# razorx89/nmfgpu

Measured on AMD Instinct MI355X. Metric: NMF MU iterations/sec, dense 10kx5k r=64, higher is better.
Workload: dtype f32; 1 GPU; configs[1]: dense random V 10000x5000, r=64, MU Frobenius, fp32; rows=10000, columns=5000, features=64, error_every=10, parallelism=single GPU

## Files before the change

nmfgpu_amd/csrc/amd_api.cpp:

```cpp
#include <hip/hip_runtime.h>

#include <algorithm>
#include <cmath>
#include <cstring>
#include <string>
#include <memory>
#include <new>
#include <vector>

#include "../../include/nmfgpu_amd.h"
#include "comm.h"
#include "engine.h"
#include "tuning.h"
#include "host_init.h"
#include "sharded.h"

using namespace nmfamd;

struct nmfamd_engine {
	int elem_bytes;
	std::unique_ptr<Engine<float>> f;
	std::unique_ptr<Engine<double>> d;
};

// ... 515 lines not shown
	const int RP = padded_rank(r);
	const long Xp = pad128(X), Yp = pad128(Y);
	const int KS = (Y + 15) / 16;
	FactorProductPlan plan; plan.th = 128; plan.xtiles = (int)(Xp / 128); plan.steps_total = KS; plan.nb = 2; plan.chunks = 1;
	plan.splits = plan_splits_x3(plan.xtiles, KS, prop.multiProcessorCount);
	DevBuf dA, dT, dF, dFb, dS, dO;
	const long slab_stride = (long)RP * Xp;
	if (dA.alloc(sizeof(float) * Xp * Yp) != hipSuccess || dT.alloc(sizeof(float) * Xp * Yp) != hipSuccess || dF.alloc(sizeof(float) * RP * Yp) != hipSuccess ||
	    dFb.alloc(3 * 16 * (size_t)(KS + 1) * (RP / 32) * 64) != hipSuccess ||
	    dS.alloc(sizeof(float) * slab_stride * plan.splits) != hipSuccess || dO.alloc(sizeof(float) * slab_stride) != hipSuccess) return NMFAMD_NO_DEVICE_MEMORY;
	if (hipMemset(dA.p, 0, sizeof(float) * Xp * Yp) != hipSuccess || hipMemset(dT.p, 0, sizeof(float) * Xp * Yp) != hipSuccess ||
	    hipMemset(dF.p, 0, sizeof(float) * RP * Yp) != hipSuccess) return NMFAMD_HIP_ERROR;
	if (hipMemcpy2D(dA.p, Xp * sizeof(float), A, lda * sizeof(float), X * sizeof(float), Y, hipMemcpyHostToDevice) != hipSuccess) return NMFAMD_HIP_ERROR;
	if (hipMemcpy2D(dF.p, RP * sizeof(float), F, ldf * sizeof(float), r * sizeof(float), Y, hipMemcpyHostToDevice) != hipSuccess) return NMFAMD_HIP_ERROR;
	const int ith = (y_tiled || x16) ? 16 : 128;
	const long tstride = y_tiled ? 16 * Xp : (x16 ? 16 * Yp : 128 * Yp);
	if (y_tiled) { if (launch_tile_transposed<float>((const float*)dA.p, Xp, X, Y, (float*)dT.p, tstride, 16, nullptr) != hipSuccess) return NMFAMD_HIP_ERROR; }
	else if (launch_tile<float>((const float*)dA.p, Xp, X, Y, (float*)dT.p, tstride, ith, false, nullptr) != hipSuccess) return NMFAMD_HIP_ERROR;
	if (launch_pack_panel_x3((const float*)dF.p, RP, Y, dFb.p, KS, nullptr) != hipSuccess) return NMFAMD_HIP_ERROR;
	if (launch_factor_product_x3(plan, (const float*)dT.p, tstride, dFb.p, RP, (float*)dS.p, slab_stride, nullptr, nullptr, nullptr, y_tiled, ith) != hipSuccess) return NMFAMD_HIP_ERROR;
	if (launch_reduce_slabs<float>((const float*)dS.p, plan.splits, slab_stride, (float*)dO.p, slab_stride, nullptr) != hipSuccess) return NMFAMD_HIP_ERROR;
	if (hipMemcpy2D(OUT, ldo * sizeof(float), dO.p, RP * sizeof(float), r * sizeof(float), X, hipMemcpyDeviceToHost) != hipSuccess) return NMFAMD_HIP_ERROR;
	if (reps > 0 && avg_us) {
		DevBuf dT2;
		if (dT2.alloc(sizeof(float) * Xp * Yp) != hipSuccess) return NMFAMD_NO_DEVICE_MEMORY;
		if (hipMemcpy(dT2.p, dT.p, sizeof(float) * Xp * Yp, hipMemcpyDeviceToDevice) != hipSuccess) return NMFAMD_HIP_ERROR;
		hipEvent_t e0, e1;
		if (hipEventCreate(&e0) != hipSuccess || hipEventCreate(&e1) != hipSuccess) return NMFAMD_HIP_ERROR;
		for (int i = 0; i < 4; ++i) (void)launch_factor_product_x3(plan, (const float*)((i & 1) ? dT2.p : dT.p), tstride, dFb.p, RP, (float*)dS.p, slab_stride, nullptr, nullptr, nullptr, y_tiled, ith);
		(void)hipEventRecord(e0, nullptr);
		for (int i = 0; i < reps; ++i) (void)launch_factor_product_x3(plan, (const float*)((i & 1) ? dT2.p : dT.p), tstride, dFb.p, RP, (float*)dS.p, slab_stride, nullptr, nullptr, nullptr, y_tiled, ith);
		(void)hipEventRecord(e1, nullptr);
		if (hipEventSynchronize(e1) != hipSuccess) return NMFAMD_HIP_ERROR;
		float ms = 0; (void)hipEventElapsedTime(&ms, e0, e1);
		*avg_us = ms * 1e3 / reps;
		(void)hipEventDestroy(e0); (void)hipEventDestroy(e1);
	}
	return hipDeviceSynchronize() == hipSuccess ? NMFAMD_OK : NMFAMD_HIP_ERROR;
}

int nmfamd_op_factor_product_x3(const float* A, long lda, int X, int Y, const float* F, long ldf, int r, float* OUT, long ldo, int reps, double* avg_us) {
	return op_factor_product_x3(A, lda, X, Y, F, ldf, r, OUT, ldo, reps, avg_us, false);
}

int nmfamd_op_factor_product_x3_ytiled(const float* A, long lda, int X, int Y, const float* F, long ldf, int r, float* OUT, long ldo, int reps, double* avg_us) {
	return op_factor_product_x3(A, lda, X, Y, F, ldf, r, OUT, ldo, reps, avg_us, true);
}


int nmfamd_tune_factor_product_x3(int X, int Y, unsigned long long* stamps_out, long stamps_capacity, long* waves) {
	if (X <= 0 || Y <= 0 || !stamps_out || !waves) return NMFAMD_INVALID_ARGUMENT;
	if (nmfamd_device_count() <= 0) return NMFAMD_NO_DEVICE;
	int dev = 0; hipDeviceProp_t prop;
	if (hipGetDevice(&dev) != hipSuccess || hipGetDeviceProperties(&prop, dev) != hipSuccess) return NMFAMD_HIP_ERROR;
	const int RP = 64;
	const long Mp = pad128(X), Np = pad128(Y);
	const int ksW = (Y + 15) / 16, ksH = (X + 15) / 16;
	FactorProductPlan planW, planH;
	planW.th = planH.th = 128; planW.nb = planH.nb = 2; planW.chunks = planH.chunks = 1;
	planW.xtiles = (int)(Mp / 128); planW.steps_total = ksW; planW.splits = plan_splits_x3(planW.xtiles, ksW, prop.multiProcessorCount);
	planH.xtiles = (int)(Np / 128); planH.steps_total = ksH; planH.splits = plan_splits_x3(planH.xtiles, ksH, prop.multiProcessorCount);
	const char* ve = tuning_env("NMFAMD_X3_VARIANT");
	const bool ytiled = ve != nullptr && std::atoi(ve) >= 30;
	const FactorProductPlan& sp = ytiled ? planH : planW;
	const long nwaves = (long)sp.xtiles * sp.splits * 4;
	if (stamps_capacity < 8 * nwaves) return NMFAMD_INVALID_ARGUMENT;
	DevBuf dA, dW, dH, dWx, dHx, dS, dT;
	const long slab_stride = (long)RP * std::max(Mp, Np);
	if (dA.alloc(sizeof(float) * Mp * Np) != hipSuccess || dW.alloc(sizeof(float) * RP * Mp) != hipSuccess || dH.alloc(sizeof(float) * RP * Np) != hipSuccess ||
	    dWx.alloc(3 * 16 * (size_t)(ksH + 1) * (RP / 32) * 64) != hipSuccess || dHx.alloc(3 * 16 * (size_t)(ksW + 1) * (RP / 32) * 64) != hipSuccess ||
	    dS.alloc(sizeof(float) * slab_stride * std::max(planW.splits, planH.splits)) != hipSuccess ||
	    dT.alloc(sizeof(unsigned long long) * 8 * nwaves) != hipSuccess) return NMFAMD_NO_DEVICE_MEMORY;
	if (launch_fill_uniform<float>((float*)dA.p, (int)Mp, (int)Mp, Np, Np, 1, nullptr) != hipSuccess) return NMFAMD_HIP_ERROR;
	if (launch_fill_uniform<float>((float*)dW.p, RP, RP, Mp, Mp, 2, nullptr) != hipSuccess) return NMFAMD_HIP_ERROR;
	if (launch_fill_uniform<float>((float*)dH.p, RP, RP, Np, Np, 3, nullptr) != hipSuccess) return NMFAMD_HIP_ERROR;
	if (launch_pack_panel_x3((const float*)dW.p, RP, X, dWx.p, ksH, nullptr) != hipSuccess) return NMFAMD_HIP_ERROR;
	if (launch_pack_panel_x3((const float*)dH.p, RP, Y, dHx.p, ksW, nullptr) != hipSuccess) return NMFAMD_HIP_ERROR;
	if (hipMemset(dT.p, 0, sizeof(unsigned long long) * 8 * nwaves) != hipSuccess) return NMFAMD_HIP_ERROR;
	const long stride = 16 * Np;
	for (int i = 0; i < 40; ++i) {
		const bool last = i == 39;
		unsigned long long* sy = last && ytiled ? (unsigned long long*)dT.p : nullptr;
		unsigned long long* sx = last && !ytiled ? (unsigned long long*)dT.p : nullptr;
		if (launch_factor_product_x3(planH, (const float*)dA.p, stride, dWx.p, RP, (float*)dS.p, slab_stride, nullptr, nullptr, sy, true, 16) != hipSuccess) return NMFAMD_HIP_ERROR;
		if (launch_factor_product_x3(planW, (const float*)dA.p, stride, dHx.p, RP, (float*)dS.p, slab_stride, nullptr, nullptr, sx, false, 16) != hipSuccess) return NMFAMD_HIP_ERROR;
	}
	if (hipMemcpy(stamps_out, dT.p, sizeof(unsigned long long) * 8 * nwaves, hipMemcpyDeviceToHost) != hipSuccess) return NMFAMD_HIP_ERROR;
	*waves = nwaves;
	return NMFAMD_OK;
}

int nmfamd_op_factor_product_f64(const double* A, long lda, int X, int Y, const double* F, long ldf, int r, double* OUT, long ldo, int use_valu, int* out_slabs) {
	return op_factor_product<double>(A, lda, X, Y, F, ldf, r, OUT, ldo, use_valu != 0, out_slabs);
}

int nmfamd_op_gram_f32(const float* P, long ldp, int r, int len, float* G, long ldg) {
	if (!P || !G || r <= 0 || len <= 0 || ldp < r || ldg < r) return NMFAMD_INVALID_ARGUMENT;
	if (nmfamd_device_count() <= 0) return NMFAMD_NO_DEVICE;
	const int RP = padded_rank(r), parts = 128;
	const long lp = pad128(len);
	DevBuf dP, dPart, dG;
	if (dP.alloc(sizeof(float) * RP * lp) != hipSuccess || dPart.alloc(sizeof(float) * (size_t)RP * RP * parts) != hipSuccess || dG.alloc(sizeof(float) * RP * RP) != hipSuccess) return NMFAMD_NO_DEVICE_MEMORY;
	if (hipMemset(dP.p, 0, sizeof(float) * RP * lp) != hipSuccess) return NMFAMD_HIP_ERROR;
	if (hipMemcpy2D(dP.p, RP * sizeof(float), P, ldp * sizeof(float), r * sizeof(float), len, hipMemcpyHostToDevice) != hipSuccess) return NMFAMD_HIP_ERROR;
	if (launch_gram<float>((const float*)dP.p, RP, len, parts, (float*)dPart.p, (float*)dG.p, nullptr) != hipSuccess) return NMFAMD_HIP_ERROR;
	if (hipMemcpy2D(G, ldg * sizeof(float), dG.p, RP * sizeof(float), r * sizeof(float), r, hipMemcpyDeviceToHost) != hipSuccess) return NMFAMD_HIP_ERROR;
	return hipDeviceSynchronize() == hipSuccess ? NMFAMD_OK : NMFAMD_HIP_ERROR;
}

int nmfamd_op_gram_f64(const double* P, long ldp, int r, int len, double* G, long ldg) {
	if (!P || !G || r <= 0 || len <= 0 || ldp < r || ldg < r) return NMFAMD_INVALID_ARGUMENT;
	if (nmfamd_device_count() <= 0) return NMFAMD_NO_DEVICE;
	const int RP = padded_rank(r, sizeof(double)), parts = 128;
	const long lp = pad128(len);
	DevBuf dP, dPart, dG;
	if (dP.alloc(sizeof(double) * RP * lp) != hipSuccess || dPart.alloc(sizeof(double) * (size_t)RP * RP * parts) != hipSuccess || dG.alloc(sizeof(double) * RP * RP) != hipSuccess) return NMFAMD_NO_DEVICE_MEMORY;
	if (hipMemcpy2D(dP.p, RP * sizeof(double), P, ldp * sizeof(double), r * sizeof(double), len, hipMemcpyHostToDevice) != hipSuccess) return NMFAMD_HIP_ERROR;
	if (launch_gram<double>((const double*)dP.p, RP, len, parts, (double*)dPart.p, (double*)dG.p, nullptr) != hipSuccess) return NMFAMD_HIP_ERROR;
	if (hipMemcpy2D(G, ldg * sizeof(double), dG.p, RP * sizeof(double), r * sizeof(double), r, hipMemcpyDeviceToHost) != hipSuccess) return NMFAMD_HIP_ERROR;
	return hipDeviceSynchronize() == hipSuccess ? NMFAMD_OK : NMFAMD_HIP_ERROR;
}

int nmfamd_op_inverse_f32(const float* A, long lda, int r, float offdiag, float diag, float* Ainv, long ldi) {
	if (!A || !Ainv || r <= 0 || lda < r || ldi < r) return NMFAMD_INVALID_ARGUMENT;
	if (nmfamd_device_count() <= 0) return NMFAMD_NO_DEVICE;
	const int RP = padded_rank(r);
	DevBuf dA, dI, dW;
	if (dA.alloc(sizeof(float) * RP * RP) != hipSuccess || dI.alloc(sizeof(float) * RP * RP) != hipSuccess || dW.alloc(sizeof(double) * 2 * (size_t)r * r) != hipSuccess) return NMFAMD_NO_DEVICE_MEMORY;
	if (hipMemcpy2D(dA.p, RP * sizeof(float), A, lda * sizeof(float), r * sizeof(float), r, hipMemcpyHostToDevice) != hipSuccess) return NMFAMD_HIP_ERROR;
	if (launch_inverse_small<float>((float*)dA.p, RP, r, (float*)dI.p, (double*)dW.p, offdiag, diag, nullptr) != hipSuccess) return NMFAMD_HIP_ERROR;
	if (hipMemcpy2D(Ainv, ldi * sizeof(float), dI.p, RP * sizeof(float), r * sizeof(float), r, hipMemcpyDeviceToHost) != hipSuccess) return NMFAMD_HIP_ERROR;
	return hipDeviceSynchronize() == hipSuccess ? NMFAMD_OK : NMFAMD_HIP_ERROR;
}

int nmfamd_op_tri_update_f32(const float* P, const float* num, const float* Q, int r, int len, const float* old_colsq, int transform_num, const float* num_colsq,
                             float theta, float frag_theta, int transform_den, float* P_out, float* pack_out, float* scale_out, float* gram_out,
                             float* gram_raw_out, float* gram_image_out, float* diag_out) {
	if (!P || !num || !Q || r <= 0 || len <= 0) return NMFAMD_INVALID_ARGUMENT;
	if (nmfamd_device_count() <= 0) return NMFAMD_NO_DEVICE;
	const int RP = padded_rank(r);
	if (!tri_kernels_available(RP)) return NMFAMD_INVALID_ARGUMENT;
	const long lp = pad128(len), KS = (len + 15) / 16;
	const size_t pack_bytes = 16 * (size_t)KS * (RP / 32) * 64;
	int dev = 0, cus = 256;
	hipDeviceProp_t prop;
	if (hipGetDevice(&dev) == hipSuccess && hipGetDeviceProperties(&prop, dev) == hipSuccess && prop.multiProcessorCount > 0) cus = prop.multiProcessorCount;
	const int parts = panel_update_parts(RP, sizeof(float), (int)lp);
	DevBuf dP, dN, dQ, dOs, dNs, dPack, dPart, dG, dSq, dStage, dScale, dQx, dDummy, dG2, dImg, dDiag;
	const size_t img_bytes = (size_t)3 * 16 * (RP / 16 + 1) * (RP / 32) * 64;
	if (dG2.alloc(sizeof(float) * RP * RP) != hipSuccess || dImg.alloc(img_bytes) != hipSuccess || dDiag.alloc(sizeof(float) * RP) != hipSuccess) return NMFAMD_NO_DEVICE_MEMORY;
	if (dP.alloc(sizeof(float) * RP * lp) != hipSuccess || dN.alloc(sizeof(float) * RP * lp) != hipSuccess || dQ.alloc(sizeof(float) * RP * RP) != hipSuccess ||
	    dOs.alloc(sizeof(float) * RP) != hipSuccess || dNs.alloc(sizeof(float) * RP) != hipSuccess || dPack.alloc(pack_bytes) != hipSuccess ||
	    dPart.alloc(sizeof(float) * (size_t)gram_tri_partial_elems(cus)) != hipSuccess || dG.alloc(sizeof(float) * RP * RP) != hipSuccess ||
	    dSq.alloc(sizeof(float) * ((size_t)parts + 16) * RP) != hipSuccess || dStage.alloc(sizeof(float) * RP * colsq_stage_parts()) != hipSuccess ||
	    dScale.alloc(sizeof(float) * RP) != hipSuccess || dDummy.alloc(sizeof(float) * RP * 4) != hipSuccess || dQx.alloc((size_t)3 * 16 * (RP / 16 + 1) * (RP / 32) * 64) != hipSuccess) return NMFAMD_NO_DEVICE_MEMORY;
	if (hipMemcpy2D(dP.p, RP * sizeof(float), P, r * sizeof(float), r * sizeof(float), len, hipMemcpyHostToDevice) != hipSuccess) return NMFAMD_HIP_ERROR;
	if (hipMemcpy2D(dN.p, RP * sizeof(float), num, r * sizeof(float), r * sizeof(float), len, hipMemcpyHostToDevice) != hipSuccess) return NMFAMD_HIP_ERROR;
	if (hipMemcpy2D(dQ.p, RP * sizeof(float), Q, r * sizeof(float), r * sizeof(float), r, hipMemcpyHostToDevice) != hipSuccess) return NMFAMD_HIP_ERROR;
	if (old_colsq && hipMemcpy(dOs.p, old_colsq, sizeof(float) * r, hipMemcpyHostToDevice) != hipSuccess) return NMFAMD_HIP_ERROR;
	if (num_colsq && hipMemcpy(dNs.p, num_colsq, sizeof(float) * r, hipMemcpyHostToDevice) != hipSuccess) return NMFAMD_HIP_ERROR;
	PanelTriExtras ex;
	ex.num_transform = transform_num != 0;
	ex.num_colsq = num_colsq ? (const float*)dNs.p : nullptr; ex.num_colsq_parts = 1;
	const float off = theta / (float)(unsigned)r, diag = (float)((1.0 - theta) + off);
	ex.num_a = diag - off; ex.num_b = off; ex.r = r;
	ex.old_colsq = old_colsq ? (const float*)dOs.p : nullptr; ex.old_colsq_parts = 1;
	ex.frag_out = dPack.p; ex.frag_KS = KS;
// ... 254 lines not shown
```

nmfgpu_amd/csrc/engine.cpp:

```cpp
#include "engine.h"
#include "tuning.h"

#include <algorithm>
#include <cmath>
#include <cstdint>
#include <cstdio>
#include <cstdlib>
#include <cstring>
#include <limits>
#include <type_traits>

namespace nmfamd {

#define HIPX(call)                                        \
	do {                                                  \
		hipError_t e__ = (call);                          \
		if (e__ != hipSuccess) return hip_fail(e__, #call); \
	} while (0)

template <typename T>
double resolve_frobenius(const std::vector<T>& vtv_sorted, std::vector<T>& htwtv, std::vector<T>& hhtwtw) {
	return std::sqrt(resolve_frobenius_squared<T>(vtv_sorted, htwtv, hhtwtw));
}
template double resolve_frobenius<float>(const std::vector<float>&, std::vector<float>&, std::vector<float>&);
// ... 161 lines not shown
		if (why != nullptr) { last_error_ = why; return ST_INVALID; }
		tiled_ = false;
		planH_.splits = planW_.splits = 1; planH_.th = planW_.th = 128;
		planH_.xtiles = (int)(pad128(n_) / 128); planW_.xtiles = (int)(pad128(m_) / 128);
	}
	if (beta_dense_) {
		tiled_ = false;
		planH_.th = planW_.th = 128;
		planH_.xtiles = (int)(pad128(n_) / 128); planW_.xtiles = (int)(pad128(m_) / 128);
		betaH_ = plan_beta_half_step(pad128(n_), pad128(m_), RP_, sizeof(T), num_cus_);
		betaW_ = plan_beta_half_step(pad128(m_), pad128(n_), RP_, sizeof(T), num_cus_);
		planH_.splits = betaH_.slabs; planW_.splits = betaW_.slabs;
	}
	if (prm_.precision > 0) {
		if (!std::is_same<T, float>::value || sparse_ || !mfma) return ST_INVALID;
		bf16_ = true;
		tiled_ = false;
		planH_.th = planW_.th = 128;
		planH_.xtiles = (int)(pad128(n_) / 128); planW_.xtiles = (int)(pad128(m_) / 128);
		ksW_ = (n_ + 15) / 16; ksH_ = (m_ + 15) / 16;
		planH_.splits = plan_splits_bf16(planH_.xtiles, ksH_, RP_, num_cus_);
		planW_.splits = plan_splits_bf16(planW_.xtiles, ksW_, RP_, num_cus_);
		if (RP_ == 256 && (alg_ == ALG_MU || alg_ == ALG_NSNMF) && tri_kernels_available(RP_)) {
			const char* e = tuning_env("NMFAMD_TRI_RIDE");
			const bool want_w = e == nullptr || (e[0] != '0' && e[0] != 'h'), want_h = e == nullptr || (e[0] != '0' && e[0] != 'w');
			if (want_w && num_cus_ > 2 * TRI_PASSENGERS) {
				FactorProductPlan t = planH_;
				t.splits = plan_splits_bf16(planH_.xtiles, ksH_, RP_, num_cus_ - TRI_PASSENGERS);
				if (bf16_product_workgroups(t) + TRI_PASSENGERS <= num_cus_) { planH_.splits = t.splits; tri_ride_w_ = true; }
			}
			tri_ride_h_ = want_h && bf16_product_workgroups(planW_) + TRI_PASSENGERS <= num_cus_;
		}
		planHb_ = planH_; planWb_ = planW_;
	}
	const size_t image_bytes = sizeof(T) * (size_t)pad128(m_) * (size_t)pad128(n_);
	const size_t mall = memory_side_cache_bytes(prop);
	const bool cache_window = mall > 0 && (double)image_bytes > 0.6 * (double)mall && (double)image_bytes < 1.12 * (double)mall && std::getenv("NMFAMD_ONE_IMAGE") == nullptr;
#ifdef NMFAMD_DIAG_BUILD
	const char* op_env = tuning_env("NMFAMD_ONE_PASS");
	const bool op_req = op_env != nullptr && std::atoi(op_env) != 0 && one_pass_allowed_ && row_blocks_ == 1 && fused_capable() && RP_ == 64 &&
	                    std::getenv("NMFAMD_GRAM_PARTIALS") == nullptr && tuning_env("NMFAMD_IMAGE_TILE128") == nullptr && onepass_available(pad128(m_), num_cus_);
#else
	const bool op_req = false;
#endif
	if (std::is_same<T, float>::value && tiled_ && !bf16_ && !sparse_ && RP_ % 64 == 0 && prm_.precision == 0 && (planH_.nb == 2 || cache_window || op_req) &&
	    tuning_env("NMFAMD_FP32_NATIVE") == nullptr) {
		planH_.nb = planW_.nb = 2;
		x3_ = true;
		planH_.th = planW_.th = 128;
		planH_.xtiles = (int)(pad128(n_) / 128); planW_.xtiles = (int)(pad128(m_) / 128);
		ksW_ = (n_ + 15) / 16; ksH_ = (m_ + 15) / 16;
		gram_ksplit_ = 1;
		if (fused_capable() && RP_ == 64 && std::getenv("NMFAMD_GRAM_PARTIALS") == nullptr) {
			const double product_us = 6.0 + (double)sizeof(T) * (double)pad128(m_) * (double)pad128(n_) / 5.0e6;
			const double pairs = (ksH_ + 2) / 2;
			while (gram_ksplit_ < GRAM_KSPLIT_MAX && 24.0 * (pairs / 317.0) / gram_ksplit_ > 0.55 * product_us) gram_ksplit_ *= 2;
			if (const char* e = tuning_env("NMFAMD_GRAM_KSPLIT")) { const int k = std::atoi(e); if (k == 1 || k == 2 || k == 4 || k == 8) gram_ksplit_ = k; }
		}
		planH_.splits = plan_splits_x3(planH_.xtiles, ksH_, num_cus_, gram_ksplit_ > 1 ? GRAM_IMAGE_TILES * gram_ksplit_ : 0);
		planW_.splits = plan_splits_x3(planW_.xtiles, ksW_, num_cus_);
		planHx_ = planH_; planWx_ = planW_;
		planHx_.steps_total = ksH_; planWx_.steps_total = ksW_;
		planHx_.nb = planWx_.nb = 2;
		size_t free_b = 0, total_b = 0;
		const size_t image_b = sizeof(T) * (size_t)pad128(m_) * (size_t)pad128(n_);
		const char* force = std::getenv("NMFAMD_ONE_IMAGE");
		one_pass_ = op_req && (force == nullptr || std::atoi(force) != 0);
		if (one_pass_) one_image_ = true;
		else if (force != nullptr) one_image_ = std::atoi(force) != 0;
		else if (cache_window) one_image_ = true;
		else if (hipMemGetInfo(&free_b, &total_b) == hipSuccess && 3 * image_b + (image_b >> 3) > free_b) one_image_ = true;
		w_col_split_ = false;
		if (RP_ == 64 && fused_capable() && !one_image_ && 2 * planW_.xtiles + GRAM_REDUCE_BLOCKS <= 2 * num_cus_) {
			w_col_split_ = ksW_ <= 80 && 4 * planW_.xtiles >= num_cus_;
			if (const char* e = tuning_env("NMFAMD_X3_COLSPLIT")) { const int v = std::atoi(e); if (v == 0) w_col_split_ = false; else if (v == 1) w_col_split_ = true; }
			if (w_col_split_) { planW_.splits = planWx_.splits = 1; planWx_.col_split = 2; }
		}
		if (const char* e = tuning_env("NMFAMD_X3_COLSPLIT")) { if (std::atoi(e) == 2 && RP_ == 64 && fused_capable()) { planHx_.col_split = planWx_.col_split = 2; w_col_split_ = true; } }
	}
	mpad_ = pad128(std::max<long>(m_, (long)planW_.xtiles * planW_.th));
	if (row_blocks_ > 1) { const long g = 128l * row_blocks_; mpad_ = ((mpad_ + g - 1) / g) * g; }
	npad_ = pad128(std::max<long>(n_, (long)planH_.xtiles * planH_.th));
	img_th_ = (one_image_ && tuning_env("NMFAMD_IMAGE_TILE128") == nullptr) ? 16 : planW_.th;
	strideV_ = (long)img_th_ * npad_;
	strideVt_ = (long)planH_.th * mpad_;
	elemsV_ = mpad_ * npad_;
	elemsVt_ = tiled_ ? (long)planH_.xtiles * strideVt_ : mpad_ * npad_;
	slab_stride_ = (long)RP_ * std::max(mpad_, npad_);
	const long slab_elems = slab_stride_ * std::max(planH_.splits, planW_.splits);
	const long panelW = (long)RP_ * mpad_, panelH = (long)RP_ * npad_, rr = (long)RP_ * RP_;

	auto dalloc = [&](T** p, long elems) -> hipError_t {
		hipError_t e = hipMalloc((void**)p, (size_t)elems * sizeof(T));
		if (e != hipSuccess) return e;
		return hipMemsetAsync(*p, 0, (size_t)elems * sizeof(T), stream_);
	};
	if (bf16_) {
		HIPX(hipMalloc(&Vb_, 16 * (size_t)planW_.xtiles * ksW_ * 256));
		HIPX(hipMalloc(&Vtb_, 16 * (size_t)planH_.xtiles * ksH_ * 256));
		{
			const size_t ks_alloc = (size_t)std::max<long>(ksH_, mpad_ / 16);
			HIPX(hipMalloc(&Wtb_, 16 * ks_alloc * (RP_ / 32) * 64));
			if (ks_alloc > (size_t)ksH_) HIPX(hipMemsetAsync((char*)Wtb_ + 16 * (size_t)ksH_ * (RP_ / 32) * 64, 0, 16 * (ks_alloc - (size_t)ksH_) * (RP_ / 32) * 64, stream_));
		}
		HIPX(hipMalloc(&Hb_, 16 * (size_t)ksW_ * (RP_ / 32) * 64));
	} else if (!sparse_) {
		if (x3_) {
			const size_t bw = 3 * 16 * (size_t)(ksH_ + 1) * (RP_ / 32) * 64, bh = 3 * 16 * (size_t)(ksW_ + 1) * (RP_ / 32) * 64;
			HIPX(hipMalloc(&Wx3_, bw));
			HIPX(hipMalloc(&Hx3_, bh));
			HIPX(hipMemsetAsync(Wx3_, 0, bw, stream_));
			HIPX(hipMemsetAsync(Hx3_, 0, bh, stream_));
		}
		HIPX(dalloc(&V_, elemsV_));
		if (!one_image_) HIPX(dalloc(&Vt_, elemsVt_));
	} else {
		HIPX(dalloc(&t_vwh_, mpad_));
		HIPX(dalloc(&t_kl_, mpad_));
		HIPX(dalloc(&rowsum_part_, (std::max(mpad_, npad_) / 128) * RP_));
		HIPX(dalloc(&sW_, RP_));
		HIPX(dalloc(&sH_, RP_));
		HIPX(dalloc(&kl_scale_, RP_));
		HIPX(hipHostMalloc((void**)&pin_kl_, sizeof(T) * (2 * (size_t)m_ + 3 * (size_t)RP_)));
		if (prm_.is_masked()) HIPX(dalloc(&msq_part_, (long)(MASKED_NORM_PARTS + 16) * RP_));
	}
	if (beta_dense_) {
		HIPX(dalloc(&t_vwh_, mpad_));
		HIPX(dalloc(&t_kl_, mpad_));
		HIPX(dalloc(&rowsum_part_, (std::max(mpad_, npad_) / 128) * RP_));
		HIPX(dalloc(&sW_, RP_));
		HIPX(dalloc(&sH_, RP_));
		HIPX(dalloc(&beta_tpart_, 2l * BETA_MAX_SLABS * mpad_));
		if (beta_ != 1) HIPX(dalloc(&beta_den_, slab_elems));
		HIPX(hipHostMalloc((void**)&pin_kl_, sizeof(T) * (2 * (size_t)m_ + 3 * (size_t)RP_)));
	}
	HIPX(dalloc(&Wt_, panelW));
	HIPX(dalloc(&H_, panelH));
	if (std::is_same<T, float>::value && panel_update_wide_available(RP_) && std::getenv("NMFAMD_FORCE_VALU") == nullptr &&
	    tuning_env("NMFAMD_WIDE_FP32_MFMA") == nullptr)
	{
		const size_t qb = 3 * 16 * (size_t)(RP_ / 16 + 1) * (RP_ / 32) * 64;
		HIPX(hipMalloc(&qx3_, qb));
		HIPX(hipMemsetAsync(qx3_, 0, qb, stream_));
	}
	HIPX(dalloc(&slabs_, slab_elems));
	HIPX(dalloc(&numW_, panelW));
	HIPX(dalloc(&G_, rr));
	HIPX(dalloc(&G2_, rr));
	HIPX(dalloc(&HHt_, rr));
	HIPX(dalloc(&Qinv_, rr));
	HIPX(dalloc(&gram_part_, rr * gram_parts_));
	HIPX(dalloc(&sumsq_part_, ((long)std::max({panel_update_parts(RP_, sizeof(T), (int)mpad_), (int)(mpad_ / panel_update_rows(RP_, sizeof(T))),
	                                           alg_ == ALG_HALS ? panel_sweep_hals_parts(RP_, sizeof(T), (int)mpad_) : 0}) + 16) * RP_));
	ps_stride_ = std::max<long>(npad_, RP_);
	HIPX(dalloc(&psN_, ps_stride_ + RP_));
	psR_ = psN_ + ps_stride_;
	HIPX(dalloc(&stage_, std::max(mpad_, npad_) * RP_));
	HIPX(hipMalloc((void**)&range_flag_, sizeof(int)));
	if constexpr (std::is_same<T, float>::value) {
		tri_ = bf16_ && tri_kernels_available(RP_) && (alg_ == ALG_MU || alg_ == ALG_NSNMF);
		if (tri_) {
			HIPX(hipMalloc((void**)&gram_tri_part_, sizeof(float) * (size_t)std::max<long>(gram_tri_partial_elems(num_cus_), (long)(TRI_PASSENGERS / 2) * 36 * 1024)));
			HIPX(hipMalloc((void**)&tri_ride_counters_, 64));
			HIPX(hipMemsetAsync(tri_ride_counters_, 0, 64, stream_));
			HIPX(dalloc(&Gw_raw_, rr));
			HIPX(dalloc(&Gh_raw_, rr));
// ... 406 lines not shown
void Engine<T>::record_begin(int kind) {
	if (!timing_ || !timing_now_) return;
	if (ev_used_ + 2 > ev_.size()) {
		for (int i = 0; i < 64; ++i) { hipEvent_t e; if (hipEventCreate(&e) != hipSuccess) return; ev_.push_back(e); }
	}
	if (ev_kind_.size() < ev_.size() / 2) ev_kind_.resize(ev_.size() / 2, 0);
	ev_kind_[ev_used_ / 2] = (char)kind;
	(void)hipEventRecord(ev_[ev_used_], stream_);
}

template <typename T>
bool Engine<T>::timed_launch_events(int kind, hipEvent_t* start, hipEvent_t* stop) {
	*start = *stop = nullptr;
	if (!timing_ || !timing_now_) return false;
	if (ev_used_ + 2 > ev_.size()) {
		for (int i = 0; i < 64; ++i) { hipEvent_t e; if (hipEventCreate(&e) != hipSuccess) return false; ev_.push_back(e); }
	}
	if (ev_kind_.size() < ev_.size() / 2) ev_kind_.resize(ev_.size() / 2, 0);
	ev_kind_[ev_used_ / 2] = (char)kind;
	*start = ev_[ev_used_]; *stop = ev_[ev_used_ + 1];
	return true;
}

template <typename T>
void Engine<T>::record_end() {
	if (!timing_ || !timing_now_ || ev_used_ + 2 > ev_.size()) return;
	(void)hipEventRecord(ev_[ev_used_ + 1], stream_);
	ev_used_ += 2;
}

template <typename T>
void Engine<T>::dominant_stats(double* total_ms, long* launches, double* pair_overhead_ms, double* kind_ms, long* kind_launches) {
	double tot = 0; long cnt = 0;
	double km[2] = {0, 0}; long kc[2] = {0, 0};
	(void)hipStreamSynchronize(stream_);
	for (size_t i = 0; i + 1 < ev_used_; i += 2) {
		float ms = 0;
		if (hipEventElapsedTime(&ms, ev_[i], ev_[i + 1]) == hipSuccess) {
			tot += ms; ++cnt;
			const int k = (i / 2 < ev_kind_.size() && ev_kind_[i / 2] != 0) ? 1 : 0;
			km[k] += ms; ++kc[k];
		}
	}
	ev_used_ = 0;
	if (total_ms) *total_ms = tot;
	if (launches) *launches = cnt;
	if (kind_ms) { kind_ms[0] = km[0]; kind_ms[1] = km[1]; }
	if (kind_launches) { kind_launches[0] = kc[0]; kind_launches[1] = kc[1]; }
	if (pair_overhead_ms) {
		double best = -1;
		if (ev_.size() >= 2) {
			for (int i = 0; i < 8; ++i) {
				(void)hipEventRecord(ev_[0], stream_);
				(void)hipEventRecord(ev_[1], stream_);
				(void)hipEventSynchronize(ev_[1]);
				float ms = 0;
				if (hipEventElapsedTime(&ms, ev_[0], ev_[1]) == hipSuccess && (best < 0 || ms < best)) best = ms;
			}
		}
		*pair_overhead_ms = best < 0 ? 0.0 : best;
	}
}

template <typename T>
GramReduceArgs Engine<T>::gram_args(bool of_w, float* G, float* scale, int normalize) const {
	GramReduceArgs rg = {of_w ? gramW_part_ : gramH_part_, (int)((of_w ? mpad_ : npad_) / 64), G, scale, normalize};
	if (gram_image_) {
		rg.partials = nullptr; rg.parts = 0; rg.image = of_w ? Wx3_ : Hx3_; rg.image_ks = of_w ? ksH_ : ksW_;
		if (of_w && normalize != 0 && wsq_part_ != nullptr) { rg.colsq_part = wsq_part_; rg.colsq_parts = (int)(mpad_ / 32); }
		if (of_w && (const void*)G == (const void*)G_ && gram_ksplit_ > 1 && Gpart_ != nullptr && (normalize == 0 || rg.colsq_part != nullptr)) { rg.ksplit = gram_ksplit_; rg.G = Gpart_; }
		else if (of_w && (const void*)G == (const void*)G_ && gram_spread_ && Gpart_ != nullptr && (normalize == 0 || rg.colsq_part != nullptr)) { rg.spread = 1; rg.G = Gpart_; rg.spread_out = G; rg.spread_counter = gram_spread_counter_; }
	}
	return rg;
}

template <typename T>
Status Engine<T>::standalone_gram(const GramReduceArgs& rg) {
	if (rg.image != nullptr) HIPX(launch_gram_image_args(rg, stream_));
	else HIPX(launch_mu64_gram_reduce(rg, stream_));
	return ST_OK;
}

template <typename T>
Status Engine<T>::mu64_update(bool is_w, const T* slabs, int S, long slab_stride, const T* Q, bool compute_error, const PeerSlabs* peers) {
	if constexpr (std::is_same<T, float>::value) {
		const float eps = std::numeric_limits<float>::epsilon();
		float* P = is_w ? Wt_ : H_;
		float* ps = ps_direct_ ? (is_w ? pin_psN_dev_ + ps_stride_ : pin_psN_dev_) : (is_w ? psR_ : psN_);
		const int len = is_w ? m_ : n_, len_pad = (int)(is_w ? mpad_ : npad_);
		void* xo = x3_ ? (is_w ? Wx3_ : Hx3_) : nullptr;
		const int xks = is_w ? ksH_ : ksW_;
		if (peers != nullptr && !gram_image_) return ST_INVALID;
		SmoothAround ns;
		ns.off = (float)prm_.theta / (float)(unsigned)r_; ns.diag = (float)((1.0 - (float)prm_.theta) + ns.off); ns.r = r_;
		const bool smooth = alg_ == ALG_NSNMF && !is_w;
		if (alg_ == ALG_NSNMF && !gram_image_) return ST_INVALID;
		if (gram_image_) HIPX(launch_mu64_update32(is_w ? 1 : 0, P, slabs, S, slab_stride, Q, scale_, eps, ps, len, len_pad, is_w ? G_ : nullptr, compute_error ? 1 : 0, stream_, xo, xks, peers,
		                                           is_w ? wsq_part_ : nullptr, (!is_w && (const void*)Q == (const void*)Gpart_) ? gram_ksplit_ : 0, (!is_w && (const void*)Q == (const void*)Gpart_) ? G_ : nullptr,
		                                           smooth ? &ns : nullptr));
		else HIPX(launch_mu64_update(is_w ? 1 : 0, P, slabs, S, slab_stride, Q, scale_, eps, ps, len, len_pad, is_w ? gramW_part_ : gramH_part_, is_w ? G_ : nullptr,
		                             compute_error ? 1 : 0, stream_, xo, xks));
	}
	return ST_OK;
}

template <typename T>
Status Engine<T>::product_h(const T* F, const GramReduceArgs* rg, bool prepacked) {
	if (sparse_) {
		if (rg) { if (Status st = standalone_gram(*rg)) return st; }
		record_begin();
		HIPX(launch_spmm_rows<T>(csc_ptr_, csc_idx_, csc_val_, F, RP_, slabs_, n_, (int)npad_, stream_));
		record_end();
		return ST_OK;
	}
	if constexpr (std::is_same<T, float>::value) {
		if (bf16_) {
			if (!prepacked) HIPX(launch_pack_panel_bf16(F, RP_, m_, Wtb_, ksH_, stream_));
			if (rg && rg->tri_frags == nullptr && planHb_.xtiles < GRAM_REDUCE_BLOCKS) { if (Status st = standalone_gram(*rg)) return st; rg = nullptr; }
			record_begin();
#ifdef NMFAMD_DIAG_BUILD
			if (unsigned long long* st = bf_stamps(0)) set_factor_product_bf16_stamps(st);
#endif
			HIPX(launch_factor_product_bf16(planHb_, Vtb_, ksH_, Wtb_, RP_, slabs_, slab_stride_, stream_, rg));
			record_end();
			return ST_OK;
		}
		if (x3_) {
			if (!prepacked) HIPX(launch_pack_panel_x3(F, RP_, m_, Wx3_, ksH_, stream_));
			if (rg && rg->wide_P == nullptr && !passengers_ride(planHx_)) { if (Status st = standalone_gram(*rg)) return st; rg = nullptr; }
			hipEvent_t e0, e1;
			const bool timed = timed_launch_events(0, &e0, &e1);
			if (one_image_) HIPX(launch_factor_product_x3(planHx_, V_, strideV_, Wx3_, RP_, slabs_, slab_stride_, stream_, rg, nullptr, true, img_th_, e0, e1));
			else HIPX(launch_factor_product_x3(planHx_, Vt_, strideVt_, Wx3_, RP_, slabs_, slab_stride_, stream_, rg, nullptr, false, 128, e0, e1));
			if (timed) timed_launch_done();
			return ST_OK;
		}
		if (tiled_) {
			if (rg && planH_.xtiles < GRAM_REDUCE_BLOCKS) { if (Status st = standalone_gram(*rg)) return st; rg = nullptr; }
			record_begin();
			HIPX(launch_factor_product_f32(planH_, Vt_, strideVt_, F, RP_, slabs_, slab_stride_, stream_, rg));
			record_end();
			return ST_OK;
		}
	}
	if constexpr (std::is_same<T, double>::value) {
		if (tiled_) {
			record_begin();
			HIPX(launch_factor_product_f64(planH_, Vt_, strideVt_, F, RP_, slabs_, slab_stride_, stream_, ride64_));
			record_end();
			return ST_OK;
		}
	}
	record_begin();
	HIPX(launch_factor_product_valu<T>(Vt_, npad_, (int)npad_, m_, F, RP_, slabs_, stream_));
	record_end();
	return ST_OK;
}

template <typename T>
Status Engine<T>::product_w(const T* F, const GramReduceArgs* rg, T* single_slab_out, bool prepacked) {
	T* dest = (single_slab_out != nullptr && planW_.splits == 1) ? single_slab_out : slabs_;
	if (sparse_) {
		if (rg) { if (Status st = standalone_gram(*rg)) return st; }
		record_begin(1);
		HIPX(launch_spmm_rows<T>(csr_ptr_, csr_idx_, csr_val_, F, RP_, dest, m_, (int)mpad_, stream_));
		record_end();
		return ST_OK;
	}
	if constexpr (std::is_same<T, float>::value) {
		if (bf16_) {
			if (!prepacked) HIPX(launch_pack_panel_bf16(F, RP_, n_, Hb_, ksW_, stream_));
			if (rg && rg->tri_frags == nullptr && planWb_.xtiles < GRAM_REDUCE_BLOCKS) { if (Status st = standalone_gram(*rg)) return st; rg = nullptr; }
			record_begin(1);
#ifdef NMFAMD_DIAG_BUILD
			if (unsigned long long* st = bf_stamps(1)) set_factor_product_bf16_stamps(st);
#endif
			HIPX(launch_factor_product_bf16(planWb_, Vb_, ksW_, Hb_, RP_, dest, slab_stride_, stream_, rg));
			record_end();
			return ST_OK;
		}
		if (x3_) {
			if (!prepacked) HIPX(launch_pack_panel_x3(F, RP_, n_, Hx3_, ksW_, stream_));
// ... 735 lines not shown
#ifdef NMFAMD_DIAG_BUILD
	if constexpr (std::is_same<T, float>::value) {
		if (!fused_ready_) { normalize_next_ = 0; fused_ready_ = true; }
		if (!wx3_valid_) { HIPX(launch_pack_panel_x3(Wt_, RP_, m_, Wx3_, ksH_, stream_)); wx3_valid_ = true; }
		GramReduceArgs rgW = gram_args(true, G_, scale_, normalize_next_);
		rgW.ksplit = 0; rgW.spread = 0; rgW.G = G_;
		if (Status s = standalone_gram(rgW)) return s;
		OnePassArgs a;
		a.V = V_; a.tile_stride = strideV_;
		a.Wx3 = Wx3_; a.G = G_; a.scale = scale_; a.ps = op_ps4_; a.ps_stride = npad_;
		if constexpr (std::is_same<T, float>::value) { a.H = H_; a.H_out = op_H2_; }
		a.slabs = op_slabs_; a.slab_stride = (long)RP_ * mpad_;
		a.hh_part = op_hh_part_; a.part_scratch = op_part_; a.hfrag_scratch = op_hfrag_;
		a.ticket = op_ctl_; a.abort_flag = op_ctl_ + 8;
		a.tile_rows = (int)(mpad_ / 16); a.w_ks = ksH_; a.n = n_; a.panels = (n_ + 31) / 32;
		a.seq = op_seq_++;
		a.compute_error = compute_error ? 1 : 0;
		a.eps = std::numeric_limits<float>::epsilon();
		a.stamps = op_stamps_;
		record_begin();
#ifdef NMFAMD_DIAG_BUILD
		HIPX(launch_mu64_onepass(a, stream_));
#else
		return ST_INVALID;
#endif
		record_end();
		std::swap(H_, op_H2_);
		HIPX(launch_reduce_partials<float>(op_hh_part_, ONEPASS_XCDS * ONEPASS_GROUP, 4096, HHt_, 4096, stream_));
		if (compute_error) HIPX(launch_reduce_partials<float>(op_ps4_, 4, npad_, psN_, n_, stream_));
		if (Status s = mu64_update(true, op_slabs_, ONEPASS_XCDS, (long)RP_ * mpad_, HHt_, compute_error)) return s;
		wx3_valid_ = x3_;
		hx3_valid_ = false;
		normalize_next_ = 1;
		w_pending_ = true;
		if (compute_error) {
			if (Status s = fetch_error_terms(n_)) return s;
			if (Status s = onepass_check()) return s;
		}
	}
#else
	(void)compute_error;
#endif
	return ST_OK;
}

template <typename T>
Status Engine<T>::onepass_check() {
#ifdef NMFAMD_DIAG_BUILD

	HIPX(hipMemcpyAsync(pin_abort_, op_ctl_ + 8, sizeof(unsigned), hipMemcpyDeviceToHost, stream_));
	HIPX(hipStreamSynchronize(stream_));
	if (op_stamps_ != nullptr) {
		std::vector<unsigned long long> h(16 * 8 * ONEPASS_XCDS * ONEPASS_GROUP);
		if (hipMemcpy(h.data(), op_stamps_, sizeof(unsigned long long) * h.size(), hipMemcpyDeviceToHost) == hipSuccess) {
			if (FILE* f = std::fopen(tuning_env("NMFAMD_ONEPASS_STAMPS"), "wb")) { std::fwrite(h.data(), sizeof(unsigned long long), h.size(), f); std::fclose(f); }
		}
	}
	if (*pin_abort_ != 0) {
		one_pass_ = false; one_pass_gave_up_ = true;
		last_error_ = "the one-pass iteration could not keep its workgroups resident (another kernel on the device?): factors are void; unset NMFAMD_ONE_PASS";
		return ST_HIP_ERROR;
	}
#endif
	return ST_OK;
}

template <typename T>
Status Engine<T>::iterate_mu64(bool compute_error) {
	if constexpr (std::is_same<T, float>::value) {
		if (one_pass_) return iterate_onepass(compute_error);
		const float eps = std::numeric_limits<float>::epsilon();
		static const bool no_direct = tuning_env("NMFAMD_ERROR_MEMCPY") != nullptr || tuning_env("NMFAMD_ERROR_COPY_KERNEL") != nullptr;
		ps_direct_ = compute_error && gram_image_ && !error_terms_stay_ && pin_psN_dev_ != nullptr && !no_direct;
		if (ps_direct_) finalize_error(false);
		struct DirectGuard { bool& f; ~DirectGuard() { f = false; } } direct_guard{ps_direct_};
		if (!fused_ready_) {
			if (!gram_image_) HIPX(launch_mu64_gram_partials(Wt_, (int)mpad_, gramW_part_, stream_));
			normalize_next_ = 0;
			fused_ready_ = true;
		}
		GramReduceArgs rgW = gram_args(true, G_, scale_, normalize_next_);
		if (h_product_ahead_) h_product_ahead_ = false;
		else if (Status s = product_h(Wt_, &rgW, x3_ && wx3_valid_)) return s;
		if (Status s = mu64_update(false, slabs_, planH_.splits, slab_stride_, rgW.ksplit > 1 ? reinterpret_cast<const T*>(Gpart_) : G_, compute_error)) return s;
		GramReduceArgs rgH = gram_args(false, HHt_, nullptr, 0);
		if (Status s = product_w(H_, &rgH, nullptr, x3_)) return s;
		if (Status s = mu64_update(true, slabs_, planW_.splits, slab_stride_, HHt_, compute_error)) return s;
		wx3_valid_ = x3_;
		hx3_valid_ = false;
		normalize_next_ = 1;
		w_pending_ = true;
		if (compute_error) {
			if (Status s = fetch_error_terms(n_)) return s;
		}
	}
	return ST_OK;
}

template <typename T>
Status Engine<T>::begin_next_iteration() {
	if constexpr (std::is_same<T, double>::value) {
		if (!fused64_capable() || f64_partial_ == nullptr || !f64_pending_ || f64_product_ahead_ || prm_.divergence != 0) return ST_OK;
		const bool sampled = timing_now_;
		timing_now_ = false;
		const Status s = fused64_product_h();
		timing_now_ = sampled;
		if (s != ST_OK) return s;
		f64_product_ahead_ = true;
		return ST_OK;
	}
	if constexpr (std::is_same<T, float>::value) {
		if (!fused_capable() || one_pass_ || !fused_ready_ || h_product_ahead_ || prm_.divergence != 0 || !x3_ || !wx3_valid_) return ST_OK;
		GramReduceArgs rgW = gram_args(true, G_, scale_, normalize_next_);
		const bool sampled = timing_now_;
		timing_now_ = false;
		const Status s = product_h(Wt_, &rgW, true);
		timing_now_ = sampled;
		if (s != ST_OK) return s;
		h_product_ahead_ = true;
	}
	return ST_OK;
}

template <typename T>
Status Engine<T>::set_hals_penalties(double l1W, double l1H, double l2W, double l2H) {
	if (const char* why = hals_penalties_fault(l1W, l1H, l2W, l2H, sizeof(T) == 4, prm_.takes_penalties(alg_ == ALG_HALS))) { last_error_ = why; return ST_INVALID; }
	prm_.l1W = (double)(T)l1W; prm_.l1H = (double)(T)l1H; prm_.l2W = (double)(T)l2W; prm_.l2H = (double)(T)l2H;
	return ST_OK;
}

template <typename T>
Status Engine<T>::iterate(bool compute_error, bool constant_w) {
	const T eps = std::numeric_limits<T>::epsilon();
	timing_now_ = timing_ && (timing_iter_++ % timing_stride_ == 0);
	if (prm_.is_masked()) return iterate_masked(compute_error, constant_w);
	if (beta_dense_) return iterate_beta(compute_error, constant_w);
	if (prm_.divergence != 0) return constant_w ? ST_INVALID : iterate_kl(compute_error);
	if (fused_capable() && !constant_w) return iterate_mu64(compute_error);
	if (fused64_capable() && !constant_w) return iterate_fused64(compute_error);
	if (f32w_scale_ != nullptr && fused32w_capable() && !constant_w) return iterate_fused32w(compute_error);
	const int norm_parts = panel_update_parts(RP_, sizeof(T), (int)mpad_);
	h_partials_unneeded_ = !constant_w;
	const Status hs = h_step_impl(compute_error);
	h_partials_unneeded_ = false;
	if (hs != ST_OK) return hs;

	const bool ls_family = alg_ == ALG_ALS || alg_ == ALG_ACLS || alg_ == ALG_AHCLS;
	int error_terms_n = n_;

	if (!(constant_w && !compute_error)) {
		const T* Fh = H_;
		bool hht_done = false;
		GramReduceArgs tri_ride = {nullptr, 0, nullptr, nullptr, 0};
		if (tri_) {
			if (Status s = tri_prepare_h(HHt_, true, !constant_w ? &tri_ride : nullptr)) return s;
			hht_done = true;
		} else if (alg_ == ALG_NSNMF) {
			const T off = (T)prm_.theta / (T)(unsigned)r_;
			const T diag = (T)((1.0 - (T)prm_.theta) + off);
			HIPX(launch_smooth_panel<T>(H_, Hs_, RP_, r_, npad_, off, diag, stream_));
			Fh = Hs_;
		}
		bool hht_rides = false;
		if constexpr (std::is_same<T, float>::value) {
			hht_rides = !constant_w && alg_ == ALG_GDCLS && x3_ && hx3_valid_ && Fh == H_ && RP_ == 64 && !gram_h_partials_ && passengers_ride(planWx_);
			if (!hht_rides && gram_h_partials_ && Fh == H_) {
				HIPX(launch_gram64_from_partials(gramH_part_, (int)(npad_ / 64), HHt_, nullptr, stream_));
				hht_done = true;
			}
		}
// ... 481 lines not shown
```

nmfgpu_amd/csrc/engine.h:

```cpp
#pragma once

#include <hip/hip_runtime.h>
#include <stdint.h>

#include <functional>
#include <vector>

#include "kernels.h"

namespace nmfamd {

enum Algorithm { ALG_MU = 0, ALG_GDCLS = 1, ALG_ALS = 2, ALG_ACLS = 3, ALG_AHCLS = 4, ALG_NSNMF = 5, ALG_HALS = 6 };

struct AlgorithmParams {
	double lambda = 0, lambdaW = 0, lambdaH = 0, alphaW = 0, alphaH = 0, theta = 0;
	double divergence = 0;
	double sparse_compute = 0;
	double precision = 0;
	double missing_values = 0;
	double l1W = 0, l1H = 0, l2W = 0, l2H = 0;
	double dense_compute = 0;
	double beta_value = 0;
	bool is_masked() const { return missing_values != 0; }
	bool is_beta_dense() const { return divergence == 2 || divergence == 3 || (divergence == 1 && dense_compute != 0); }
// ... 116 lines not shown
	int n() const { return n_; }
	int r() const { return r_; }
	int rp() const { return RP_; }
	bool error_terms_per_factor_row() const { return alg_ != ALG_MU && alg_ != ALG_NSNMF && alg_ != ALG_HALS; }
	int algorithm() const { return alg_; }
	long mpad() const { return mpad_; }
	long npad() const { return npad_; }
	int slabs_h() const { return planH_.splits; }
	int slabs_w() const { return planW_.splits; }
	int resident_images() const { return sparse_ ? 0 : (one_image_ ? 1 : 2); }
	int product_kernel() const { return beta_dense_ ? 6 : sparse_ ? 5 : bf16_ ? 1 : x3_ ? 2 : !tiled_ ? 4 : (sizeof(T) == 8 ? 3 : 0); }
	const char* last_error() const { return last_error_; }

	Status debug_read(int which, T* out, long count);

private:
	Status hip_fail(hipError_t e, const char* what);
	Status h_step_impl(bool compute_error);
	Status product_h(const T* F, const GramReduceArgs* rg = nullptr, bool prepacked = false);
	Status product_w(const T* F, const GramReduceArgs* rg = nullptr, T* single_slab_out = nullptr, bool prepacked = false);
	bool fused_capable() const;
	bool fused32w_capable() const;
	Status iterate_fused32w(bool compute_error);
	bool fused64_capable() const;
	Status iterate_fused64(bool compute_error);
	bool gram_from_update() const;
	Status iterate_mu64(bool compute_error);
	Status iterate_onepass(bool compute_error);
	Status onepass_check();
	Status materialize_w(bool whole_panel = true);
	Status ensure_w_rows();
	Status normalize_w(bool from_gram_partials, int norm_parts);
	Status normal_inverse(T* A, T offdiag, T diag);
	Status normal_inverse_fork(T* A, T offdiag, T diag);
	Status normal_inverse_join();
	bool passengers_ride(const FactorProductPlan& plan) const;
	bool inverse_rides(const FactorProductPlan& plan) const;
	Status finish_upload(T* Vcol);
	Status upload_triplets(std::vector<int>& rows, std::vector<int>& cols, std::vector<T>& vals);
	Status upload_sparse_device(int format, const T* values, const int* a, const int* b, long nnz, int base, bool* fallback);
	Status setup_kl_blocks();
	bool sparse_setup_on_device_ = false;
	Status iterate_kl(bool compute_error);
	Status iterate_masked(bool compute_error, bool constant_w);
	Status masked_refuses(const char* what);
	Status iterate_beta(bool compute_error, bool constant_w);
	Status beta_refuses(const char* what);
	Status beta_check_values(const T* values, long count, long ld, long rows);
	Status fetch_error_terms(int count_n);
	void finalize_error(bool resolve);
	void record_begin(int kind = 0);
	void record_end();
	bool timed_launch_events(int kind, hipEvent_t* start, hipEvent_t* stop);
	void timed_launch_done() { ev_used_ += 2; }

	int m_, n_, r_, RP_, alg_;
	int row_blocks_ = 1;
	AlgorithmParams prm_;
	long mpad_, npad_;
	long strideV_ = 0, strideVt_ = 0, elemsV_ = 0, elemsVt_ = 0;
	int num_cus_ = 256;
	hipStream_t stream_ = nullptr;
	hipStream_t aux_ = nullptr;
	hipEvent_t ev_fork_ = nullptr, ev_join_ = nullptr;
	bool overlap_inverse_ = false;
	bool tiled_ = false;
	const char* last_error_ = "";

	T *V_ = nullptr, *Vt_ = nullptr;
	T *Wt_ = nullptr, *H_ = nullptr;
	T *Ws_ = nullptr, *Hs_ = nullptr;
	T *slabs_ = nullptr;
	T *numW_ = nullptr;
	T *Wold_ = nullptr;
	T *rowdot_part_ = nullptr;
	T *G_ = nullptr, *G2_ = nullptr, *HHt_ = nullptr, *Qinv_ = nullptr, *gram_part_ = nullptr;
	T *sumsq_part_ = nullptr;
	bool bf16_ = false;
	void *Vb_ = nullptr, *Vtb_ = nullptr, *Wtb_ = nullptr, *Hb_ = nullptr;
	int ksW_ = 0, ksH_ = 0;
	FactorProductPlan planHb_, planWb_;
	bool x3_ = false;
	bool one_image_ = false;
	int img_th_ = 128;
	bool wx3_valid_ = false, hx3_valid_ = false;
	void *Wx3_ = nullptr, *Hx3_ = nullptr;
	void* qx3_ = nullptr;
	FactorProductPlan planHx_, planWx_;
	bool sparse_ = false;
	long nnz_ = 0;
	int *csr_ptr_ = nullptr, *csr_idx_ = nullptr, *csc_ptr_ = nullptr, *csc_idx_ = nullptr, *csc_from_csr_ = nullptr;
	T *csr_val_ = nullptr, *csc_val_ = nullptr, *q_ = nullptr, *q2_ = nullptr;
	T *t_vwh_ = nullptr, *t_kl_ = nullptr, *rowsum_part_ = nullptr, *sW_ = nullptr, *sH_ = nullptr;
	int kl_blocks_w_ = 1, kl_blocks_h_ = 1;
	int *csr_bptr_ = nullptr, *csc_bptr_ = nullptr;
	T *kl_part_ = nullptr, *kl_tpart_ = nullptr;
	double sum_v_ = 0, kl_ = 0;
	T* pin_kl_ = nullptr;
	bool kl_pending_ = false, kl_unresolved_ = false;
	std::vector<T> h_klrow_, h_sW_, h_sH_;
	T* msq_part_ = nullptr;
	bool masked_pending_ = false, masked_unresolved_ = false;
	bool beta_dense_ = false, beta_uploaded_ = false;
	double beta_ = 1;
	BetaPlan betaH_, betaW_;
	T *beta_den_ = nullptr, *beta_tpart_ = nullptr;
	bool beta_pending_ = false, beta_unresolved_ = false;
	float *gramW_part_ = nullptr, *gramH_part_ = nullptr, *scale_ = nullptr, *Graw64_ = nullptr;
	bool w_col_split_ = false;
	bool gram_spread_ = false;
	unsigned* gram_spread_counter_ = nullptr;
	int gram_ksplit_ = 1;
	float* Gpart_ = nullptr;
	float* wsq_part_ = nullptr;
	bool fused_ready_ = false, w_pending_ = false;
	bool h_product_ahead_ = false;
	bool gram_image_ = false;
	GramReduceArgs gram_args(bool of_w, float* G, float* scale, int normalize) const;
	Status standalone_gram(const GramReduceArgs& rg);
	Status mu64_update(bool is_w, const T* slabs, int S, long slab_stride, const T* Q, bool compute_error, const PeerSlabs* peers = nullptr);
	bool gram_w_ready_ = false;
	bool tri_ = false;
	unsigned* tri_ride_counters_ = nullptr;
	bool tri_ride_w_ = false, tri_ride_h_ = false;
	bool wtb_valid_ = false;
	bool tri_scale_pending_ = false;
	bool tri_scale_from_gram_ = false;
	bool sole_rank_ = false;
	T* kl_scale_ = nullptr;
	bool kl_scale_pending_ = false;
	bool kl_sw_ready_ = false;
	bool kl_err_iter_ = false;
	long err_total_columns_ = 0;
	Status kl_h_step();
	Status kl_w_products(T* exchange, bool compute_error);
	Status kl_w_finish(const T* exchange, bool compute_error);
	bool tri_w_den_bf16_ = true;
	bool hb_valid_ = false;
	const T* tri_trace_scale() const { return (tri_ && tri_scale_pending_) ? reinterpret_cast<const T*>(colsq_) : nullptr; }
	bool tri_gw_ready_ = false;
	bool tri_rows_cover_ = false;
	bool w_rows_stale_ = false;
	std::function<Status()> w_gather_hook_;
	int colsq_parts_ = 1;
	float *gram_tri_part_ = nullptr, *Gw_raw_ = nullptr, *Gh_raw_ = nullptr, *colsq_ = nullptr;
	bool qx3_holds_g_ = false, qx3_holds_hht_ = false;
	void tri_smoothing(T* offdiag, T* diag) const;
	Status tri_prepare_w(GramReduceArgs* ride = nullptr);
	Status tri_prepare_h(T* hht, bool local_q, GramReduceArgs* ride = nullptr);
	Status tri_update_w(const T* num, int S, long stride, const T* hht);
	bool f32w_pending_ = false;
	float* f32w_scale_ = nullptr;
	int f32w_ride_h_ = 0, f32w_ride_w_ = 0;
	bool f64_pending_ = false;
	bool f64_product_ahead_ = false;
	Status fused64_product_h();
	double *f64_scale_ = nullptr, *f64_partial_ = nullptr;
	unsigned* f64_counters_ = nullptr;
	int *f64_items_h_ = nullptr, *f64_items_w_ = nullptr;
	int f64_slices_h_ = 0, f64_slices_w_ = 0;
	const GramRideF64* ride64_ = nullptr;
	unsigned long long* f64_stamps_ = nullptr;
	bool gram_h_partials_ = false;
	bool h_partials_unneeded_ = false;
	int normalize_next_ = 0;
	T *psN_ = nullptr, *psR_ = nullptr;
	long ps_stride_ = 0;
	double* inv_work_ = nullptr;
	T* stage_ = nullptr;
	int* range_flag_ = nullptr;
	long slab_stride_ = 0;
	int gram_parts_ = 128;
	FactorProductPlan planH_, planW_;
	bool one_pass_allowed_ = true, one_pass_ = false, one_pass_gave_up_ = false;
	void *op_part_ = nullptr, *op_hfrag_ = nullptr;
	unsigned *op_ctl_ = nullptr;
	float *op_slabs_ = nullptr, *op_hh_part_ = nullptr, *op_ps4_ = nullptr;
	T* op_H2_ = nullptr;
	unsigned op_seq_ = 0;
	unsigned* pin_abort_ = nullptr;
	unsigned long long* op_stamps_ = nullptr;

	T *pin_psN_ = nullptr, *pin_psR_ = nullptr;
	bool error_terms_stay_ = false;
	bool ps_last_direct_ = false;
	bool ps_direct_ = false;
	T* pin_psN_dev_ = nullptr;
	hipEvent_t err_event_ = nullptr;
	bool err_pending_ = false, err_unresolved_ = false;
	int err_count_ = 0;
	std::vector<T> h_vtv_, h_psN_, h_psR_;
	double frob_ = 0, frob2_ = 0, rmsd_ = 0;

	bool timing_ = false;
	int timing_stride_ = 1;
	long timing_iter_ = 0;
	bool timing_now_ = false;
	std::vector<hipEvent_t> ev_;
	std::vector<char> ev_kind_;
	size_t ev_used_ = 0;
};

template <typename T>
// ... 6 lines not shown
```

nmfgpu_amd/csrc/kernels.h:

```cpp
#pragma once

#include <hip/hip_runtime.h>
#include <stddef.h>
#include <stdint.h>

#include <atomic>
#include <vector>

namespace nmfamd {

struct FactorProductPlan {
	int th;
	int xtiles;
	int steps_total;
	int splits;
	int nb;
	int chunks;
	int xhalves = 0;
	int half_tiles = 0;
	int col_split = 0;
};

FactorProductPlan plan_factor_product(int X, int Y, int RP, int num_cus);

inline hipError_t allow_dynamic_lds(const void* kernel, int bytes, std::atomic<unsigned long long>& done) {
	int dev = 0;
	hipError_t e = hipGetDevice(&dev);
	if (e != hipSuccess) return e;
	if (dev >= 0 && dev < 64 && ((done.load(std::memory_order_acquire) >> dev) & 1ull)) return hipSuccess;
	e = hipFuncSetAttribute(kernel, hipFuncAttributeMaxDynamicSharedMemorySize, bytes);
	if (e == hipSuccess && dev >= 0 && dev < 64) done.fetch_or(1ull << dev, std::memory_order_release);
	return e;
}

struct GramReduceArgs {
	const float* partials;
	int parts;
	float* G;
	float* scale;
	int normalize;
	const float* inv_a = nullptr;
	float* inv_out = nullptr;
	float inv_offdiag = 0.f, inv_diag = 0.f;
	int inv_r = 0;
	const void* image = nullptr;
	int image_ks = 0;
	const float* colsq_part = nullptr;
	int colsq_parts = 0;
	int ksplit = 0;
	int spread = 0;
	float* spread_out = nullptr;
	unsigned* spread_counter = nullptr;
	const void* tri_frags = nullptr;
	int tri_ks = 0;
	void* tri_x3 = nullptr;
	float* tri_diag = nullptr;
	float* tri_partial = nullptr;
	unsigned* tri_counters = nullptr;
	const float* wide_P = nullptr;
	int wide_len = 0, wide_parts = 0;
	float* wide_partial = nullptr;
};
constexpr int GRAM_REDUCE_BLOCKS = 16;
constexpr int TRI_PASSENGERS = 32;
constexpr int GRAM_IMAGE_TILES = 10;
constexpr int GRAM_SPREAD_SLICES = 3;
constexpr int GRAM_KSPLIT_MAX = 8;

hipError_t launch_factor_product_f32(const FactorProductPlan& p, const float* A, long tile_stride, const float* F, int RP,
                                     float* slabs, long slab_stride, hipStream_t stream, const GramReduceArgs* rg = nullptr);

template <typename T>
hipError_t launch_tile(const T* src, long ld, int X, int Y, T* dst, long tile_stride, int th, bool untile, hipStream_t stream);
template <typename T>
hipError_t launch_tile_transposed(const T* src, long ld, int I, int J, T* dst, long tile_stride, int th, hipStream_t stream);

hipError_t launch_factor_product_f32_stamped(const FactorProductPlan& p, const float* A, long lda, const float* F, int RP,
                                             float* slabs, long slab_stride, unsigned long long* stamps, hipStream_t stream);

hipError_t launch_mu64_gram_partials(const float* P, int len_pad, float* partial, hipStream_t stream);
hipError_t launch_mu64_gram_reduce(const GramReduceArgs& rg, hipStream_t stream);
hipError_t launch_mu64_update(int is_w, float* P, const float* slabs, int S, long slab_stride, const float* Q, const float* scale,
                              float eps, float* ps, int len_valid, int len_pad, float* gram_partial, const float* Gprev,
                              int compute_error, hipStream_t stream, void* x3_out = nullptr, int x3_ks = 0);
constexpr int PEER_SLABS_MAX = 16;
struct PeerSlabs { const float* p[PEER_SLABS_MAX]; int count; };
struct SmoothAround { float off, diag; int r; };
hipError_t launch_mu64_update32(int is_w, float* P, const float* slabs, int S, long slab_stride, const float* Q, const float* scale,
                                float eps, float* ps, int len_valid, int len_pad, const float* Gprev, int compute_error, hipStream_t stream,
                                void* x3_out, int x3_ks, const PeerSlabs* peers = nullptr, float* colsq_part = nullptr, int qsplit = 0, float* q_out = nullptr,
                                const SmoothAround* ns = nullptr);
hipError_t launch_sum_peers(const PeerSlabs& src, float* out, int count, hipStream_t stream);
hipError_t launch_gram_from_image(const void* image, int image_ks, float* G, float* scale, int normalize, hipStream_t stream, const float* colsq_part = nullptr, int colsq_parts = 0);
hipError_t launch_gram_image_args(const GramReduceArgs& rg, hipStream_t stream);
hipError_t launch_mu64_apply_scale(float* P, int len_pad, const float* scale, hipStream_t stream, void* x3_out = nullptr, int x3_ks = 0);
hipError_t launch_gram64_from_partials(const float* partials, int parts, float* G, float* scale, hipStream_t stream);
hipError_t launch_gram64_normalize_all(const float* partials, int parts, float* Graw, float* G, float* scale, float* P, int len_pad, void* x3_out, int x3_ks, hipStream_t stream);
hipError_t launch_gram64_reduce_scale_all(const float* gram_part, int parts, const float* sumsq_part, int sq_parts, float* G, float* scale, float* P, int len_pad,
                                          void* x3_out, int x3_ks, hipStream_t stream);

template <typename T>
hipError_t launch_factor_product_valu(const T* A, long lda, int Xpad, int Y, const T* F, int RP, T* out, hipStream_t stream);

template <typename T>
hipError_t launch_reduce_slabs(const T* slabs, int S, long slab_stride, T* out, long count, hipStream_t stream);

template <typename T>
hipError_t launch_gram(const T* P, int RP, int len, int parts, T* partial, T* G, hipStream_t stream);

enum PanelMode { PANEL_MU = 0, PANEL_LS = 1, PANEL_SET = 2 };
struct PanelTriExtras {
	bool num_transform = false;
	const float* num_colsq = nullptr;
	int num_colsq_parts = 0;
	float num_a = 1.0f, num_b = 0.0f;
	int r = 0;
	bool den_transform = false;
	float den_a = 1.0f, den_b = 0.0f;
	const float* den_colsq = nullptr;
	int den_colsq_parts = 0;
	const float* old_colsq = nullptr;
	int old_colsq_parts = 0;
	bool old_as_bf16 = false;
	void* frag_out = nullptr;
	long frag_KS = 0;
	float frag_a = 1.0f, frag_b = 0.0f;
};
int panel_update_rows(int RP, size_t elem);
int panel_update_parts(int RP, size_t elem, int len_pad);

hipError_t launch_gram64_f32(const float* P, int len, int parts, float* partial, float* G, hipStream_t stream);
hipError_t launch_panel_update64_f32(int mode, float* P, const float* slabs, int S, long slab_stride, const float* Q, int len_pad,
                                     float eps, float* ps, int len_valid, float* sumsq_part, float* num_out, hipStream_t stream);
hipError_t launch_panel_update64_lds_f32(int mode, float* P, const float* slabs, int S, long slab_stride, const float* Q, int len_pad,
                                         float eps, float* ps, int len_valid, float* sumsq_part, float* num_out, hipStream_t stream,
                                         float* gram_partial = nullptr, void* x3_out = nullptr, int x3_ks = 0);
bool panel_update_delivers_gram(int RP, size_t elem);
bool panel_update_wide_available(int RP);
bool panel_update_long_available(int RP, int len_pad);
hipError_t launch_panel_update_long_mu(const float* P_in, float* P_out, const float* slabs, int S, long slab_stride, const void* q_split, int RP, int len_pad,
                                       float eps, float* ps, int len_valid, float* sumsq_part, hipStream_t stream, const PanelTriExtras* tri = nullptr);
bool gram_wide_available(int RP);
hipError_t launch_gram_wide_f32(const float* P, int RP, int len, int parts, float* partial, float* G, hipStream_t stream);
struct PanelFusedF32 {
	const float* old_scale = nullptr;
	int h_side = 0;
	const float* scale = nullptr;
	int smooth = 0;
	float off = 0.f, diag = 1.f;
	int r = 0;
	float* smooth_out = nullptr;
	void* x3_out = nullptr;
	long x3_ks = 0;
};
hipError_t launch_panel_update_wide_f32(int mode, float* P, const float* slabs, int S, long slab_stride, const float* Q, int RP, int len_pad,
                                        float eps, float* ps, int len_valid, float* sumsq_part, float* num_out, hipStream_t stream,
                                        void* q_split = nullptr, const PanelTriExtras* tri = nullptr, const PanelFusedF32* fused = nullptr);
hipError_t launch_gram_reduce_x3(const float* partial, int parts, int RP, float* G, void* qx3, const float* sumsq_part, int sq_parts, float* scale_out, hipStream_t stream);
int gram_wide_fused_parts(int RP, int len, int parts);
hipError_t launch_gram_wide_fused_f32(const float* P, int RP, int len, int parts, float* partial, float* G, void* qx3, const float* sumsq_part, int sq_parts,
                                      float* scale_out, hipStream_t stream);
template <typename T>
hipError_t launch_reduce_partials(const T* partial, int parts, long stride, T* out, long count, hipStream_t stream);
template <typename T>
hipError_t launch_normalize_panel_v2(T* P, int RP, int len_pad, T* sumsq_part, int parts, hipStream_t stream);

template <typename T>
hipError_t launch_panel_update(int mode, T* P, const T* slabs, int S, long slab_stride, const T* Q, int RP, int len_pad,
                               T eps, T* ps, int len_valid, T* sumsq_part, T* num_out, hipStream_t stream, T* gram_partial = nullptr,
                               void* x3_out = nullptr, int x3_ks = 0,
                               void* q_split = nullptr,
                               const PanelTriExtras* tri = nullptr);

bool panel_sweep_hals_available(int RP, size_t elem);
// ... 33 lines not shown
template <typename T>
hipError_t launch_column_sumsq(const T* V, long ldv, int rows, int cols, T* ps, hipStream_t stream, int* range_flag = nullptr);

template <typename T>
hipError_t launch_densify(int format, const T* values, const int* ptr, const int* idx, const int* idx2, long nnz, int outer, int base,
                          T* V, long ldv, int rows, int cols, hipStream_t stream);

template <typename T>
hipError_t launch_fill_uniform(T* P, int RP, int r, long len, long len_pad, uint64_t seed, hipStream_t stream, long y_first = 0);

FactorProductPlan plan_factor_product_f64(int X, int Y, int RP, int num_cus);
struct GramRideF64 {
	const double* P;
	int len;
	int slices;
	double* partial;
	unsigned* counters;
	double* G;
	const double* sumsq_part;
	int sumsq_parts;
	double* scale_out;
	const int* items;
	int stop;
	unsigned long long* stamps;
};
int gram_ride_f64_workgroups(int RP, int slices);
hipError_t launch_factor_product_f64(const FactorProductPlan& p, const double* A, long tile_stride, const double* F, int RP,
                                     double* slabs, long slab_stride, hipStream_t stream, const GramRideF64* ride = nullptr);
void gram_ride_f64_items(const FactorProductPlan& p, int RP, int slices, std::vector<int>& items);

struct PanelFusedF64 {
	const double* old_scale;
	int h_side;
	const double* scale;
	int smooth;
	double off, diag;
	int r;
	double* smooth_out;
	const double* trace_a;
	const double* trace_b;
	const double* trace_scale;
	double* trace_out;
	int trace_r;
	unsigned long long* stamps;
};
inline int panel_fused_f64_extra_workgroups(const PanelFusedF64* fx) { return (fx != nullptr && fx->trace_out != nullptr) ? (fx->trace_r + 3) / 4 : 0; }
hipError_t launch_panel_update64_f64(int mode, double* P, const double* slabs, int S, long slab_stride, const double* Q, int len_pad,
                                     double eps, double* ps, int len_valid, double* sumsq_part, double* num_out, hipStream_t stream, const PanelFusedF64* fused = nullptr);

hipError_t launch_gram_f64(const double* P, int RP, int len, int parts, double* partial, double* G, hipStream_t stream);
bool panel_update_wide_f64_available(int RP);
hipError_t launch_panel_update_wide_f64(int mode, double* P, const double* slabs, int S, long slab_stride, const double* Q, int RP, int len_pad,
                                        double eps, double* ps, int len_valid, double* sumsq_part, double* num_out, hipStream_t stream, const PanelFusedF64* fused = nullptr);

hipError_t launch_pack_stream_bf16(const float* src, long ld, int X, int Y, bool transposed, void* dst, int xtiles, int KS, hipStream_t stream);
hipError_t launch_pack_panel_bf16(const float* P, int RP, int len, void* dst, int KS, hipStream_t stream);

bool tri_kernels_available(int RP);
hipError_t launch_finish_panel_bf16(float* P, int RP, int r, long row0, long rows, const float* colsq, int colsq_parts, float offdiag, float diag, void* dst, long KS, hipStream_t stream);
int colsq_stage_parts();
hipError_t launch_colsq_stage(const float* part, int RP, int parts, float* staged, float* final_sum, hipStream_t stream);
hipError_t launch_gram_tri(const float* P, int RP, int len, int max_parts, float* partial, float* G, int num_cus, hipStream_t stream);
long gram_tri_partial_elems(int max_parts);
hipError_t launch_gram_tri_bf16(const void* frags, int RP, long KS, int max_parts, float* partial, float* G, const float* colsq, int colsq_parts, int num_cus, hipStream_t stream);
hipError_t launch_gram_tri_bf16_image(const void* frags, int RP, long KS, int max_parts, float* partial, float* G, void* x3_out, float* diag_out, int num_cus, hipStream_t stream);
hipError_t launch_scale_panel_tri(float* P, int RP, long rows, const float* colsq, int colsq_parts, float* scale_out, hipStream_t stream);
hipError_t launch_smooth_gram(const float* G, float* Gs, int RP, int r, float offdiag, float diag, void* x3_out, hipStream_t stream);
hipError_t launch_finish_and_gram(const float* P_in, float* P_out, int RP, int r, long rows, int len, const float* colsq, int colsq_parts, float offdiag, float diag,
                                  void* dst, long KS, int max_parts, float* partial, float* G, int num_cus, hipStream_t stream);
hipError_t launch_factor_product_bf16(const FactorProductPlan& p, const void* A, int KS, const void* F, int RP,
                                      float* slabs, long slab_stride, hipStream_t stream, const GramReduceArgs* rg = nullptr);
int plan_splits_bf16(int xtiles, int KS, int RP, int num_cus);
int bf16_product_workgroups(const FactorProductPlan& p);
#ifdef NMFAMD_DIAG_BUILD
void set_factor_product_bf16_stamps(unsigned long long* stamps);
#endif

hipError_t launch_pack_panel_x3(const float* P, int RP, int len, void* dst, int KS, hipStream_t stream);
hipError_t launch_factor_product_x3(const FactorProductPlan& p, const float* A, long tile_stride, const void* F, int RP,
                                    float* slabs, long slab_stride, hipStream_t stream, const GramReduceArgs* rg = nullptr,
                                    unsigned long long* stamps = nullptr, bool y_tiled = false, int image_tile = 128,
                                    hipEvent_t ev_start = nullptr, hipEvent_t ev_stop = nullptr);
int plan_splits_x3(int xtiles, int KS, int num_cus, int reserve = 0);

struct OnePassArgs {
	const float* V; long tile_stride;
	const void* Wx3;
	const float* G;
	const float* scale;
	const float* H;
	float* H_out;
	float* ps; long ps_stride;
	float* slabs; long slab_stride;
	float* hh_part;
	void* part_scratch;
	void* hfrag_scratch;
	unsigned* ticket;
	unsigned* abort_flag;
	int tile_rows;
	int w_ks;
	int n;
	int panels;
	unsigned seq;
	int compute_error;
	float eps;
	unsigned long long* stamps = nullptr;
};
constexpr int ONEPASS_SLOTS = 4;
constexpr int ONEPASS_GROUP = 32;
constexpr int ONEPASS_XCDS = 8;
constexpr int ONEPASS_TILES_PER_WAVE = 5;
constexpr size_t onepass_part_bytes() { return (size_t)ONEPASS_XCDS * ONEPASS_SLOTS * ONEPASS_GROUP * 256 * 64; }
constexpr size_t onepass_hfrag_bytes() { return (size_t)ONEPASS_XCDS * ONEPASS_SLOTS * 64 * 32 * 8; }
bool onepass_available(long mpad, int num_cus);
hipError_t launch_mu64_onepass(const OnePassArgs& a, hipStream_t stream);

template <typename T>
hipError_t launch_spmm_rows(const int* ptr, const int* idx, const T* val, const T* P, int RP, T* out, int rows, int rows_pad, hipStream_t stream);
template <typename T>
hipError_t launch_sddmm_quotient(const int* ptr, const int* idx, const T* val, const T* A, const T* B, int RP, T eps,
                                 T* q, T* t_vwh, T* t_kl, int rows, hipStream_t stream);
template <typename T>
hipError_t launch_kl_fused(const int* ptr, const int* idx, const T* val, const T* A, const T* B, int RP, T eps,
                           T* out, T* t_vwh, T* t_kl, int rows, int rows_pad, hipStream_t stream, int blocks = 1, long out_stride = 0,
                           const T* a_scale = nullptr);
template <typename T>
hipError_t launch_permute(const T* src, const int* perm, T* dst, long count, hipStream_t stream);
template <typename T>
hipError_t launch_panel_rowsum(const T* P, int RP, int len_pad, T* partial, T* sums, hipStream_t stream);
template <typename T>
hipError_t launch_kl_update(T* P, const T* num, const T* den, int RP, int len_pad, T eps, T* sumsq_part, hipStream_t stream, int parts = 1, long part_stride = 0,
                            T* sum_part = nullptr,
                            const T* scale = nullptr);
template <typename T>
hipError_t launch_kl_sums(const T* sum_part, const T* sumsq_part, int parts, int RP, T* sums, hipStream_t stream, T* scale_out = nullptr);

constexpr int MASKED_NORM_PARTS = 2048;
int masked_norm_parts(int rows);
template <typename T>
hipError_t launch_masked_half_step(const int* ptr, const int* idx, const T* val, T* A, const T* B, int RP, T eps, bool update,
                                   T* t_res, T* sumsq_part, int rows, hipStream_t stream);

constexpr int BETA_MAX_SLABS = 16;
struct BetaPlan { int bo = 0, kt = 0, slabs = 0, tiles = 0, tiles_per_slab = 0; };
bool beta_half_step_available(int RP);
BetaPlan plan_beta_half_step(long out_pad, long red_pad, int RP, size_t elem_bytes, int num_cus, int force_slabs = 0);
template <typename T>
hipError_t launch_beta_fused(const T* X, long ldx, const T* A, const T* B, int RP, double beta, bool update, bool terms, T eps, const BetaPlan& plan,
                             T* num_part, T* den_part, long part_stride, T* tf_part, T* td_part, long t_stride,
                             int out_pad, int out_valid, int red_valid, hipStream_t stream);
template <typename T>
hipError_t launch_beta_update(T* A, const T* num_part, const T* den_part, long part_stride, int slabs, const T* dsum, int RP, int r, int out_pad, int out_valid, T eps,
                              double beta, T l1, T l2, bool update, T* sumsq_part, T* sum_part, const T* tf_part, const T* td_part, long t_stride, T* t_frob,
                              T* t_div, hipStream_t stream);

hipError_t launch_sp_expand(int format, const int* a, const int* b, long nnz, int outer, int base, int m, int n, int* row, int* col, int* flags, hipStream_t stream);
hipError_t launch_sp_histogram_scan(const int* key, long count, int segments, int* counts, int* ptr, int* maxlen, hipStream_t stream);
long sp_segment_sort_capacity();
hipError_t launch_sp_scatter_sort(const int* key, long count, int segments, const int* ptr, int* fill, int* items, const int* minor, int maxlen, hipStream_t stream);
template <typename T>
hipError_t launch_sp_gather_csr(const int* order, const int* row, const int* col, const T* val, long nnz, int* csr_idx, T* csr_val, int* rowq, hipStream_t stream);
template <typename T>
hipError_t launch_sp_gather_csc(const int* cq, const int* rowq, const T* csr_val, long nnz, int* csc_idx, T* csc_val, hipStream_t stream);
template <typename T>
hipError_t launch_sp_col_sumsq(const int* csc_ptr, const T* csc_val, int n, T* vtv, double* colsum, hipStream_t stream);
hipError_t launch_sp_boundaries(const int* ptr, const int* idx, int rows, long range, int blocks, int* bp, hipStream_t stream);
// ... 3 lines not shown
```

nmfgpu_amd/csrc/kernels_mu64.hip:

```cpp
#include <hip/hip_runtime.h>
#include <stdint.h>

#include "kernels.h"
#include "split3.h"
#include "gram_image.h"

namespace nmfamd {

typedef float f32x16 __attribute__((ext_vector_type(16)));

template <bool IS_W>
__global__ __launch_bounds__(256) void k_mu64_update(
	float* __restrict__ P, const float* __restrict__ slabs, int S, long slab_stride,
	const float* __restrict__ Q, const float* __restrict__ scale, float eps,
	float* __restrict__ ps, int len_valid, float* __restrict__ gram_partial,
	const float* __restrict__ Gprev, int compute_error, bf16x8* __restrict__ x3_out, int x3_ks) {
	__shared__ __attribute__((aligned(16))) float s_num[64][68];
	__shared__ __attribute__((aligned(16))) float s_old[64][68];
	__shared__ float s_ps[2][64];
	const int tid = threadIdx.x;
	const int wave = tid >> 6, lane = tid & 63;
	const int half = lane >> 5, l31 = lane & 31;
	const int ct = wave & 1, mb = wave >> 1;
	const long tile = (long)blockIdx.x * 64 * 64;
	const int c4 = (4 * tid) & 63;
	const int yl0 = tid >> 4;

	f32x4 nl[4], ol[4];
	{
		f32x4 t[7][4];
#pragma unroll
		for (int j = 0; j < 4; ++j) {
			const long e = tile + 4 * (tid + 256 * j);
			nl[j] = *reinterpret_cast<const f32x4*>(slabs + e);
			ol[j] = *reinterpret_cast<const f32x4*>(P + e);
#pragma unroll
			for (int u = 0; u < 7; ++u) {
				const int k = 1 + u < S ? 1 + u : 0;
				t[u][j] = *reinterpret_cast<const f32x4*>(slabs + (long)k * slab_stride + e);
			}
		}
#pragma unroll
		for (int u = 0; u < 7; ++u)
			if (1 + u < S) {
#pragma unroll
				for (int j = 0; j < 4; ++j) nl[j] += t[u][j];
			}
		for (int k0 = 8; k0 < S; k0 += 7) {
#pragma unroll
			for (int j = 0; j < 4; ++j)
#pragma unroll
				for (int u = 0; u < 7; ++u) {
					const int k = k0 + u < S ? k0 + u : 0;
					t[u][j] = *reinterpret_cast<const f32x4*>(slabs + (long)k * slab_stride + tile + 4 * (tid + 256 * j));
				}
#pragma unroll
			for (int u = 0; u < 7; ++u)
				if (k0 + u < S) {
#pragma unroll
					for (int j = 0; j < 4; ++j) nl[j] += t[u][j];
				}
		}
	}
	const f32x4 sc = *reinterpret_cast<const f32x4*>(scale + c4);
	float qa[32];
#pragma unroll
	for (int cb = 0; cb < 2; ++cb)
#pragma unroll
		for (int q = 0; q < 4; ++q)
#pragma unroll
			for (int gi = 0; gi < 4; ++gi) qa[cb * 16 + q * 4 + gi] = Q[(long)(32 * cb + 8 * q + 4 * half + gi) * 64 + 32 * mb + l31];
#pragma unroll
	for (int j = 0; j < 4; ++j) {
		if (IS_W) ol[j] *= sc; else nl[j] *= sc;
		*reinterpret_cast<f32x4*>(&s_num[yl0 + 16 * j][c4]) = nl[j];
		*reinterpret_cast<f32x4*>(&s_old[yl0 + 16 * j][c4]) = ol[j];
	}
	__syncthreads();

	const int yrow = ct * 32 + l31;
	f32x4 oldv[2][4], numv[4];
#pragma unroll
	for (int cb = 0; cb < 2; ++cb)
#pragma unroll
		for (int q = 0; q < 4; ++q) oldv[cb][q] = *reinterpret_cast<const f32x4*>(&s_old[yrow][32 * cb + 8 * q + 4 * half]);
#pragma unroll
	for (int q = 0; q < 4; ++q) numv[q] = *reinterpret_cast<const f32x4*>(&s_num[yrow][32 * mb + 8 * q + 4 * half]);
	f32x16 acc;
// ... 11 lines not shown
#pragma unroll
	for (int q = 0; q < 4; ++q) {
		f32x4 o;
#pragma unroll
		for (int gi = 0; gi < 4; ++gi) {
			const float old = mb == 0 ? oldv[0][q][gi] : oldv[1][q][gi];
			o[gi] = old * numv[q][gi] / (acc[4 * q + gi] + eps);
			psum += o[gi] * numv[q][gi];
		}
		*reinterpret_cast<f32x4*>(&s_num[yrow][32 * mb + 8 * q + 4 * half]) = o;
	}
	if (!IS_W && compute_error) {
		psum += __shfl_xor(psum, 32);
		if (half == 0) s_ps[mb][yrow] = psum;
	}
	if (IS_W && compute_error && blockIdx.x == 0) {
		for (int d = wave * 16; d < wave * 16 + 16; ++d) {
			float v = Q[(long)lane * 64 + d] * Gprev[(long)d * 64 + lane];
			for (int w = 32; w > 0; w >>= 1) v += __shfl_xor(v, w);
			if (lane == 0) ps[d] = v;
		}
	}
	__syncthreads();
	if (!IS_W && compute_error && tid < 64) {
		const int ycol = blockIdx.x * 64 + tid;
		if (ycol < len_valid) ps[ycol] = s_ps[0][tid] + s_ps[1][tid];
	}

#pragma unroll
	for (int j = 0; j < 4; ++j)
		*reinterpret_cast<f32x4*>(P + tile + 4 * (tid + 256 * j)) = *reinterpret_cast<const f32x4*>(&s_num[yl0 + 16 * j][c4]);
	if (x3_out != nullptr) {
#pragma unroll
		for (int i = 0; i < 2; ++i) {
			const int slot = tid + 256 * i;
			const int r = slot & 31, h = (slot >> 5) & 1, nb = (slot >> 6) & 1, kk = slot >> 7;
			const long ks = 4l * blockIdx.x + kk;
			if (ks < x3_ks) {
				float v[8];
#pragma unroll
				for (int j = 0; j < 8; ++j) {
					const int yl = 16 * kk + 8 * h + j;
					v[j] = blockIdx.x * 64 + yl < len_valid ? s_num[yl][32 * nb + r] : 0.f;
				}
				store_split3(x3_out, ks, 2, nb, h, r, v);
			}
		}
	}
	const int ab = wave >> 1, bb = wave & 1;
	f32x16 g;
#pragma unroll
	for (int i = 0; i < 16; ++i) g[i] = 0.f;
#pragma unroll 8
	for (int x = 0; x < 64; x += 2) {
		const float a = s_num[x + half][ab * 32 + l31];
		const float b = s_num[x + half][bb * 32 + l31];
		g = __builtin_amdgcn_mfma_f32_32x32x2f32(a, b, g, 0, 0, 0);
	}
	float* out = gram_partial + (long)blockIdx.x * 4096;
#pragma unroll
	for (int q = 0; q < 4; ++q)
#pragma unroll
		for (int gi = 0; gi < 4; ++gi) out[(long)(ab * 32 + gi + 8 * q + 4 * half) * 64 + bb * 32 + l31] = g[4 * q + gi];
}

hipError_t launch_mu64_update(int is_w, float* P, const float* slabs, int S, long slab_stride, const float* Q, const float* scale,
                              float eps, float* ps, int len_valid, int len_pad, float* gram_partial, const float* Gprev,
                              int compute_error, hipStream_t stream, void* x3_out, int x3_ks) {
	dim3 grid(len_pad / 64), block(256);
	bf16x8* xo = reinterpret_cast<bf16x8*>(x3_out);
	if (is_w) hipLaunchKernelGGL((k_mu64_update<true>), grid, block, 0, stream, P, slabs, S, slab_stride, Q, scale, eps, ps, len_valid, gram_partial, Gprev, compute_error, xo, x3_ks);
	else hipLaunchKernelGGL((k_mu64_update<false>), grid, block, 0, stream, P, slabs, S, slab_stride, Q, scale, eps, ps, len_valid, gram_partial, Gprev, compute_error, xo, x3_ks);
	return hipGetLastError();
}

#ifndef U32_Q_EARLY
#define U32_Q_EARLY 0
#endif
template <bool IS_W, int U = 7, int QS = 1, bool NS = false>
__global__ __launch_bounds__(256) void k_mu64_update32(
	float* __restrict__ P, const float* __restrict__ slabs, int S, long slab_stride,
	const float* __restrict__ Q, const float* __restrict__ scale, float eps,
	float* __restrict__ ps, int len_valid, const float* __restrict__ Gprev, int compute_error, bf16x8* __restrict__ x3_out, int x3_ks, PeerSlabs peers,
	float* __restrict__ colsq_part, int qsplit, float* __restrict__ q_out, float ns_a_arg, float ns_b_arg, int ns_r) {
	static_assert(!(NS && IS_W), "the smoothing matrix rides the H update only");
	typedef float f32x4v __attribute__((ext_vector_type(4)));
	__shared__ __attribute__((aligned(16))) float s_num[32][68];
	__shared__ __attribute__((aligned(16))) float s_old[32][68];
	__shared__ __attribute__((aligned(16))) float s_sm[NS ? 32 : 1][68];
	__shared__ float s_ps[4][32];
	__shared__ float s_dsum[NS ? 4 : 1][32], s_osum[NS ? 4 : 1][32];
	const float ns_a = NS ? in_vgpr(ns_a_arg) : 1.f, ns_b = NS ? in_vgpr(ns_b_arg) : 0.f;
	const int tid = threadIdx.x;
	const int wave = tid >> 6, lane = tid & 63;
	const int q = lane >> 4, l15 = lane & 15;
	const long tile = (long)blockIdx.x * 32 * 64;
	const int c4 = (4 * tid) & 63;
	const int yl0 = tid >> 4;

	if (peers.count > 0) S = peers.count;
	if (peers.count > 1) __builtin_amdgcn_fence(__ATOMIC_ACQUIRE, "");
	auto slab_at = [&](int k) -> const float* { return peers.count > 0 ? peers.p[k] : slabs + (long)k * slab_stride; };
	f32x4v qa[4];
	f32x4v qs[QS > 1 ? QS - 1 : 1][4];
	f32x4v nl[2], ol[2];
	{
		f32x4v t[U][2];
#pragma unroll
		for (int j = 0; j < 2; ++j) {
			const long e = tile + 4 * (tid + 256 * j);
			nl[j] = *reinterpret_cast<const f32x4v*>(slab_at(0) + e);
			ol[j] = *reinterpret_cast<const f32x4v*>(P + e);
#pragma unroll
			for (int u = 0; u < U; ++u) {
				const int k = 1 + u < S ? 1 + u : 0;
				t[u][j] = *reinterpret_cast<const f32x4v*>(slab_at(k) + e);
			}
		}
		if (QS > 1 || U32_Q_EARLY) {
			__builtin_amdgcn_sched_barrier(0);
#pragma unroll
			for (int u = 0; u < 4; ++u) qa[u] = *reinterpret_cast<const f32x4v*>(Q + (long)(16 * wave + l15) * 64 + 16 * q + 4 * u);
#pragma unroll
			for (int k = 1; k < QS; ++k)
#pragma unroll
				for (int u = 0; u < 4; ++u) qs[k - 1][u] = *reinterpret_cast<const f32x4v*>(Q + (long)k * 4096 + (long)(16 * wave + l15) * 64 + 16 * q + 4 * u);
			__builtin_amdgcn_sched_barrier(0);
		}
#pragma unroll
		for (int u = 0; u < U; ++u)
			if (1 + u < S) {
#pragma unroll
				for (int j = 0; j < 2; ++j) nl[j] += t[u][j];
			}
		for (int k0 = 1 + U; k0 < S; k0 += U) {
#pragma unroll
			for (int j = 0; j < 2; ++j)
#pragma unroll
				for (int u = 0; u < U; ++u) {
					const int k = k0 + u < S ? k0 + u : 0;
					t[u][j] = *reinterpret_cast<const f32x4v*>(slab_at(k) + tile + 4 * (tid + 256 * j));
				}
#pragma unroll
			for (int u = 0; u < U; ++u)
				if (k0 + u < S) {
#pragma unroll
					for (int j = 0; j < 2; ++j) nl[j] += t[u][j];
				}
		}
	}
	const f32x4v sc = *reinterpret_cast<const f32x4v*>(scale + c4);
	if (QS == 1 && !U32_Q_EARLY) {
#pragma unroll
		for (int u = 0; u < 4; ++u) qa[u] = *reinterpret_cast<const f32x4v*>(Q + (long)(16 * wave + l15) * 64 + 16 * q + 4 * u);
	}
	if (!IS_W && QS > 1) {
#pragma unroll
		for (int k = 1; k < QS; ++k)
#pragma unroll
			for (int u = 0; u < 4; ++u) qa[u] += qs[k - 1][u];
		const float srow = scale[16 * wave + l15];
#pragma unroll
		for (int u = 0; u < 4; ++u) {
			const f32x4v scol = *reinterpret_cast<const f32x4v*>(scale + 16 * q + 4 * u);
			qa[u] = (qa[u] * scol) * srow;
			if (blockIdx.x == 0 && q_out != nullptr) *reinterpret_cast<f32x4v*>(q_out + (long)(16 * wave + l15) * 64 + 16 * q + 4 * u) = qa[u];
		}
	}
// ... 6 lines not shown
#pragma unroll
			for (int w = 1; w < 16; w <<= 1) { sn += __shfl_xor(sn, w); so += __shfl_xor(so, w); }
			f32x4v sm;
#pragma unroll
			for (int g = 0; g < 4; ++g) {
				const bool in = c4 + g < ns_r;
				nl[j][g] = in ? ns_a * nl[j][g] + ns_b * sn : 0.f;
				sm[g] = in ? ns_a * ol[j][g] + ns_b * so : 0.f;
			}
			*reinterpret_cast<f32x4v*>(&s_sm[yl0 + 16 * j][c4]) = sm;
		}
		*reinterpret_cast<f32x4v*>(&s_num[yl0 + 16 * j][c4]) = nl[j];
		*reinterpret_cast<f32x4v*>(&s_old[yl0 + 16 * j][c4]) = ol[j];
	}
	__syncthreads();

	f32x4v ob[2][4];
#pragma unroll
	for (int yt = 0; yt < 2; ++yt)
#pragma unroll
		for (int u = 0; u < 4; ++u) ob[yt][u] = *reinterpret_cast<const f32x4v*>(NS ? &s_sm[16 * yt + l15][16 * q + 4 * u] : &s_old[16 * yt + l15][16 * q + 4 * u]);
	f32x4v acc[2] = {{0.f, 0.f, 0.f, 0.f}, {0.f, 0.f, 0.f, 0.f}};
#pragma unroll
	for (int u = 0; u < 4; ++u)
#pragma unroll
		for (int g = 0; g < 4; ++g) {
			acc[0] = __builtin_amdgcn_mfma_f32_16x16x4f32(qa[u][g], ob[0][u][g], acc[0], 0, 0, 0);
			acc[1] = __builtin_amdgcn_mfma_f32_16x16x4f32(qa[u][g], ob[1][u][g], acc[1], 0, 0, 0);
		}
	f32x4v sq = {0.f, 0.f, 0.f, 0.f};
	if (NS) {
#pragma unroll
		for (int yt = 0; yt < 2; ++yt) {
			float v = (acc[yt][0] + acc[yt][1]) + (acc[yt][2] + acc[yt][3]);
			v += __shfl_xor(v, 16);
			v += __shfl_xor(v, 32);
			if (q == 0) s_dsum[wave][16 * yt + l15] = v;
		}
		__syncthreads();
#pragma unroll
		for (int yt = 0; yt < 2; ++yt) {
			const int y = 16 * yt + l15;
			const float tsum = ((s_dsum[0][y] + s_dsum[1][y]) + s_dsum[2][y]) + s_dsum[3][y];
#pragma unroll
			for (int g = 0; g < 4; ++g) acc[yt][g] = ns_a * acc[yt][g] + ns_b * tsum;
		}
	}
#pragma unroll
	for (int yt = 0; yt < 2; ++yt) {
		const int y = 16 * yt + l15;
		const f32x4v oldv = *reinterpret_cast<const f32x4v*>(&s_old[y][16 * wave + 4 * q]);
		const f32x4v numv = *reinterpret_cast<const f32x4v*>(&s_num[y][16 * wave + 4 * q]);
		f32x4v o;
		float psum = 0.f;
#pragma unroll
		for (int g = 0; g < 4; ++g) {
			o[g] = oldv[g] * numv[g] / (acc[yt][g] + eps);
			psum += o[g] * numv[g];
			if (IS_W) sq[g] += o[g] * o[g];
		}
		*reinterpret_cast<f32x4v*>(&s_num[y][16 * wave + 4 * q]) = o;
		if (NS) {
			float v = (o[0] + o[1]) + (o[2] + o[3]);
			v += __shfl_xor(v, 16);
			v += __shfl_xor(v, 32);
			if (q == 0) s_osum[wave][y] = v;
		}
		if (!IS_W && compute_error) {
			psum += __shfl_xor(psum, 16);
			psum += __shfl_xor(psum, 32);
			if (q == 0) s_ps[wave][y] = psum;
		}
	}
	if (IS_W && colsq_part != nullptr) {
#pragma unroll
		for (int g = 0; g < 4; ++g) {
			float v = sq[g];
			v += __shfl_xor(v, 1); v += __shfl_xor(v, 2); v += __shfl_xor(v, 4); v += __shfl_xor(v, 8);
			sq[g] = v;
		}
		if (l15 == 0) *reinterpret_cast<f32x4v*>(colsq_part + (long)blockIdx.x * 64 + 16 * wave + 4 * q) = sq;
	}
	if (IS_W && compute_error && wave == 0) {
		for (int d = blockIdx.x; d < 64; d += gridDim.x) {
			float v = Q[(long)lane * 64 + d] * Gprev[(long)d * 64 + lane];
			for (int w = 32; w > 0; w >>= 1) v += __shfl_xor(v, w);
			if (lane == 0) ps[d] = v;
		}
	}
	__syncthreads();
	if (!IS_W && compute_error && tid < 32) {
		const int ycol = blockIdx.x * 32 + tid;
		if (ycol < len_valid) ps[ycol] = ((s_ps[0][tid] + s_ps[1][tid]) + s_ps[2][tid]) + s_ps[3][tid];
	}
#pragma unroll
	for (int j = 0; j < 2; ++j)
		*reinterpret_cast<f32x4v*>(P + tile + 4 * (tid + 256 * j)) = *reinterpret_cast<const f32x4v*>(&s_num[yl0 + 16 * j][c4]);
	{
		const int r = tid & 31, h = (tid >> 5) & 1, nb = (tid >> 6) & 1, kk = tid >> 7;
		const long ks = 2l * blockIdx.x + kk;
		if (ks < x3_ks) {
			float v[8];
#pragma unroll
			for (int j = 0; j < 8; ++j) {
				const int yl = 16 * kk + 8 * h + j;
				float x = s_num[yl][32 * nb + r];
				if (NS) x = 32 * nb + r < ns_r ? ns_a * x + ns_b * (((s_osum[0][yl] + s_osum[1][yl]) + s_osum[2][yl]) + s_osum[3][yl]) : 0.f;
				v[j] = blockIdx.x * 32 + yl < len_valid ? x : 0.f;
			}
			store_split3(x3_out, ks, 2, nb, h, r, v);
		}
	}
}

template <bool IS_W, int U, int QS, bool NS = false>
static void launch_update32_inst(dim3 grid, hipStream_t stream, float* P, const float* slabs, int S, long slab_stride, const float* Q, const float* scale, float eps, float* ps,
                                 int len_valid, const float* Gprev, int compute_error, bf16x8* xo, int x3_ks, const PeerSlabs& peers, float* colsq_part, float* q_out,
                                 const SmoothAround* ns = nullptr) {
	hipLaunchKernelGGL((k_mu64_update32<IS_W, U, QS, NS>), grid, dim3(256), 0, stream, P, slabs, S, slab_stride, Q, scale, eps, ps, len_valid, Gprev, compute_error, xo, x3_ks, peers,
	                   colsq_part, QS, q_out, NS ? ns->diag - ns->off : 1.f, NS ? ns->off : 0.f, NS ? ns->r : 0);
}

hipError_t launch_mu64_update32(int is_w, float* P, const float* slabs, int S, long slab_stride, const float* Q, const float* scale,
                                float eps, float* ps, int len_valid, int len_pad, const float* Gprev, int compute_error, hipStream_t stream,
                                void* x3_out, int x3_ks, const PeerSlabs* peers, float* colsq_part, int qsplit, float* q_out, const SmoothAround* ns) {
	if (x3_out == nullptr || len_pad % 32 != 0 || (qsplit > 1 && is_w) || (qsplit > 1 && qsplit != 2 && qsplit != 4 && qsplit != 8)) return hipErrorInvalidValue;
	if (ns != nullptr && (is_w || ns->r < 1 || ns->r > 64)) return hipErrorInvalidValue;
	PeerSlabs pa = {};
	if (peers != nullptr) {
		if (peers->count < 1 || peers->count > PEER_SLABS_MAX) return hipErrorInvalidValue;
		pa = *peers;
		S = peers->count;
	}
	dim3 grid(len_pad / 32);
	bf16x8* xo = reinterpret_cast<bf16x8*>(x3_out);
#define NMFAMD_U32(ISW, UU, QQ) launch_update32_inst<ISW, UU, QQ>(grid, stream, P, slabs, S, slab_stride, Q, scale, eps, ps, len_valid, Gprev, compute_error, xo, x3_ks, pa, colsq_part, q_out)
#define NMFAMD_U32NS(UU, QQ) launch_update32_inst<false, UU, QQ, true>(grid, stream, P, slabs, S, slab_stride, Q, scale, eps, ps, len_valid, Gprev, compute_error, xo, x3_ks, pa, colsq_part, q_out, ns)
	if (ns != nullptr) {
		if (S > 8) { if (qsplit == 2) NMFAMD_U32NS(13, 2); else if (qsplit == 4) NMFAMD_U32NS(13, 4); else if (qsplit == 8) NMFAMD_U32NS(13, 8); else NMFAMD_U32NS(13, 1); }
		else { if (qsplit == 2) NMFAMD_U32NS(7, 2); else if (qsplit == 4) NMFAMD_U32NS(7, 4); else if (qsplit == 8) NMFAMD_U32NS(7, 8); else NMFAMD_U32NS(7, 1); }
#undef NMFAMD_U32NS
		return hipGetLastError();
	}
	if (is_w) { if (S > 8) NMFAMD_U32(true, 13, 1); else NMFAMD_U32(true, 7, 1); }
	else if (S > 8) { if (qsplit == 2) NMFAMD_U32(false, 13, 2); else if (qsplit == 4) NMFAMD_U32(false, 13, 4); else if (qsplit == 8) NMFAMD_U32(false, 13, 8); else NMFAMD_U32(false, 13, 1); }
	else { if (qsplit == 2) NMFAMD_U32(false, 7, 2); else if (qsplit == 4) NMFAMD_U32(false, 7, 4); else if (qsplit == 8) NMFAMD_U32(false, 7, 8); else NMFAMD_U32(false, 7, 1); }
#undef NMFAMD_U32
	return hipGetLastError();
}

__global__ __launch_bounds__(256) void k_sum_peers(PeerSlabs src, float* __restrict__ out, int count) {
	__builtin_amdgcn_fence(__ATOMIC_ACQUIRE, "");
	const int i = 4 * (blockIdx.x * 256 + threadIdx.x);
	if (i >= count) return;
	f32x4 s = *reinterpret_cast<const f32x4*>(src.p[0] + i);
	for (int k = 1; k < src.count; ++k) s += *reinterpret_cast<const f32x4*>(src.p[k] + i);
	*reinterpret_cast<f32x4*>(out + i) = s;
}

hipError_t launch_sum_peers(const PeerSlabs& src, float* out, int count, hipStream_t stream) {
	if (src.count < 1 || src.count > PEER_SLABS_MAX || count % 4 != 0) return hipErrorInvalidValue;
	hipLaunchKernelGGL(k_sum_peers, dim3((unsigned)((count / 4 + 255) / 256)), dim3(256), 0, stream, src, out, count);
	return hipGetLastError();
}

__global__ __launch_bounds__(256) void k_gram_image(GramReduceArgs rg) {
	__shared__ __attribute__((aligned(16))) float lds[GRAM_IMAGE_LDS_FLOATS];
	gram_image_block(rg, blockIdx.x, lds);
}

hipError_t launch_gram_image_args(const GramReduceArgs& rg, hipStream_t stream) {
	if (rg.image == nullptr || rg.ksplit > GRAM_KSPLIT_MAX || (rg.ksplit > 1 && rg.normalize != 0 && rg.colsq_part == nullptr)) return hipErrorInvalidValue;
	hipLaunchKernelGGL(k_gram_image, dim3(rg.ksplit > 1 ? GRAM_IMAGE_TILES * rg.ksplit : GRAM_REDUCE_BLOCKS), dim3(256), 0, stream, rg);
	return hipGetLastError();
}

hipError_t launch_gram_from_image(const void* image, int image_ks, float* G, float* scale, int normalize, hipStream_t stream, const float* colsq_part, int colsq_parts) {
	GramReduceArgs rg = {nullptr, 0, G, scale, normalize};
	rg.image = image; rg.image_ks = image_ks;
	rg.colsq_part = colsq_part; rg.colsq_parts = colsq_parts;
	hipLaunchKernelGGL(k_gram_image, dim3(GRAM_REDUCE_BLOCKS), dim3(256), 0, stream, rg);
	return hipGetLastError();
}

__global__ __launch_bounds__(256) void k_mu64_gram_partials(const float* __restrict__ P, float* __restrict__ partial) {
	const int wave = threadIdx.x >> 6, lane = threadIdx.x & 63;
	const int half = lane >> 5, l31 = lane & 31;
	const int ab = wave >> 1, bb = wave & 1;
	const float* p = P + (long)blockIdx.x * 64 * 64;
	f32x16 g;
#pragma unroll
	for (int i = 0; i < 16; ++i) g[i] = 0.f;
#pragma unroll 8
	for (int x = 0; x < 64; x += 2) {
		const float a = p[(long)(x + half) * 64 + ab * 32 + l31];
		const float b = p[(long)(x + half) * 64 + bb * 32 + l31];
		g = __builtin_amdgcn_mfma_f32_32x32x2f32(a, b, g, 0, 0, 0);
	}
	float* out = partial + (long)blockIdx.x * 4096;
#pragma unroll
	for (int q = 0; q < 4; ++q)
#pragma unroll
		for (int gi = 0; gi < 4; ++gi) out[(long)(ab * 32 + gi + 8 * q + 4 * half) * 64 + bb * 32 + l31] = g[4 * q + gi];
}

hipError_t launch_mu64_gram_partials(const float* P, int len_pad, float* partial, hipStream_t stream) {
	hipLaunchKernelGGL(k_mu64_gram_partials, dim3(len_pad / 64), dim3(256), 0, stream, P, partial);
	return hipGetLastError();
}

__global__ __launch_bounds__(512) void k_mu64_gram_reduce(GramReduceArgs rg) {
	__shared__ float lds[64 + 512];
	const int tid = threadIdx.x, blk = blockIdx.x;
	float* s_scale = lds;
	float* s_tmp = lds + 64;
	const int parts = rg.parts;
	if (rg.normalize) {
		if (tid < 128) {
			const int c = tid & 63, g = tid >> 6;
			const int p0 = (parts * g) / 2, p1 = (parts * (g + 1)) / 2;
			float sum = 0.f;
			for (int p = p0; p < p1; p += 8) {
				float v[8];
#pragma unroll
				for (int u = 0; u < 8; ++u) v[u] = rg.partials[(long)(p + u < p1 ? p + u : p0) * 4096 + c * 65];
#pragma unroll
				for (int u = 0; u < 8; ++u)
					if (p + u < p1) sum += v[u];
			}
			s_tmp[g * 64 + c] = sum;
		}
		__syncthreads();
		if (tid < 64) {
			const float d = s_tmp[tid] + s_tmp[64 + tid];
			s_scale[tid] = d > 0.f ? 1.0f / sqrtf(d) : 1.0f;
		}
	} else if (tid < 64) {
		s_scale[tid] = 1.0f;
	}
	__syncthreads();
	{
		const int el = tid & 255, g = tid >> 8;
		const int e = blk * 256 + el;
		const int p0 = (parts * g) / 2, p1 = (parts * (g + 1)) / 2;
		float sum = 0.f;
		for (int p = p0; p < p1; p += 8) {
			float v[8];
// ... 189 lines not shown
```

nmfgpu_amd/csrc/kernels_x3.hip:

```cpp
#include <hip/hip_runtime.h>
#include <hip/hip_ext.h>
#include <stdint.h>

#include <algorithm>
#include <type_traits>
#include <cstdlib>

#include "kernels.h"
#include "tuning.h"
#include "split3.h"
#include "inverse_gj64.h"
#include "gram_image.h"
#include "gram_wide.h"

namespace nmfamd {

#ifndef NMFAMD_XCD_REMAP
#define NMFAMD_XCD_REMAP 1
#endif
constexpr bool XCD_REMAP = NMFAMD_XCD_REMAP != 0;

#ifndef X3_RING_X
#define X3_RING_X 2
#endif
#ifndef X3_EPILOGUE_ONE_ROUND
#define X3_EPILOGUE_ONE_ROUND 1
#endif
#ifndef X3_DEAL_TURNS
#define X3_DEAL_TURNS 0
#endif
#ifndef X3_RING_Y
#define X3_RING_Y 2
#endif

typedef float f32x16 __attribute__((ext_vector_type(16)));

__global__ __launch_bounds__(256) void k_pack_panel_x3(const float* __restrict__ P, int RP, int NBT, int len, bf16x8* __restrict__ dst, long frags) {
	const long f = (long)blockIdx.x * 256 + threadIdx.x;
	if (f >= frags) return;
	const int r = (int)(f & 31), h = (int)((f >> 5) & 1);
	const long t = f >> 6;
	const int nb = (int)(t % NBT);
	const long ks = t / NBT;
	float v[8];
#pragma unroll
	for (int j = 0; j < 8; ++j) {
		const long y = 16 * ks + 8 * h + j;
		v[j] = y < len ? P[y * RP + 32 * nb + r] : 0.f;
	}
	store_split3(dst, ks, NBT, nb, h, r, v);
}

hipError_t launch_pack_panel_x3(const float* P, int RP, int len, void* dst, int KS, hipStream_t stream) {
	const int NBT = RP / 32;
	const long frags = (long)(KS + 1) * NBT * 64;
	hipLaunchKernelGGL(k_pack_panel_x3, dim3((unsigned)((frags + 255) / 256)), dim3(256), 0, stream, P, RP, NBT, len, reinterpret_cast<bf16x8*>(dst), frags);
	return hipGetLastError();
}

template <int NT>
__device__ inline void gram_reduce_block_x3(const GramReduceArgs& rg, int blk, float* lds) {
	constexpr int NG = NT / 64;
	const int tid = threadIdx.x;
	const int g = tid >> 6, l = tid & 63;
	float* s_scale = lds;
	float* s_tmp = lds + 64;
	const int parts = rg.parts;
	const int p0 = (parts * g) / NG, p1 = (parts * (g + 1)) / NG;
	if (rg.normalize) {
		const float* dp = rg.partials + l * 65;
		float sum = 0.f;
		int p = p0;
		for (; p + 8 <= p1; p += 8) {
			float v[8];
#pragma unroll
			for (int u = 0; u < 8; ++u) v[u] = dp[(long)(p + u) * 4096];
#pragma unroll
			for (int u = 0; u < 8; ++u) sum += v[u];
		}
		for (; p < p1; ++p) sum += dp[(long)p * 4096];
		s_tmp[g * 64 + l] = sum;
		__syncthreads();
		if (tid < 64) {
			float d = s_tmp[tid];
#pragma unroll
			for (int k = 1; k < NG; ++k) d += s_tmp[k * 64 + tid];
			s_scale[tid] = d > 0.f ? 1.0f / sqrtf(d) : 1.0f;
		}
	} else if (tid < 64) {
		s_scale[tid] = 1.0f;
	}
	__syncthreads();
	{
		const float* ep = rg.partials + blk * 256 + 4 * l;
		f32x4 sum = {0.f, 0.f, 0.f, 0.f};
		int p = p0;
		for (; p + 8 <= p1; p += 8) {
			f32x4 v[8];
#pragma unroll
			for (int u = 0; u < 8; ++u) v[u] = *reinterpret_cast<const f32x4*>(ep + (long)(p + u) * 4096);
#pragma unroll
			for (int u = 0; u < 8; ++u) sum += v[u];
		}
		for (; p < p1; ++p) sum += *reinterpret_cast<const f32x4*>(ep + (long)p * 4096);
		*reinterpret_cast<f32x4*>(s_tmp + g * 256 + 4 * l) = sum;
	}
	__syncthreads();
	if (tid < 256) {
		const int e = blk * 256 + tid;
		float v = s_tmp[tid];
#pragma unroll
		for (int k = 1; k < NG; ++k) v += s_tmp[k * 256 + tid];
		rg.G[e] = (v * s_scale[e & 63]) * s_scale[e >> 6];
	}
	if (blk == 0 && tid < 64 && rg.scale) rg.scale[tid] = s_scale[tid];
}

template <int D, int X3_WAVES, int DIAG = 0, int NBW = 2, bool TR = false, int IMG = 128, bool YLDS = false, bool R32 = false, bool ODD = false>
__global__ __launch_bounds__(64 * X3_WAVES, NBW == 1 ? 2 : 1) void k_factor_product_x3(
	const float* __restrict__ A, long tile_stride,
	const bf16x8* __restrict__ F, int NBT,
	float* __restrict__ slabs, long slab_stride, int RP,
	int steps_total, int xtiles, int splits, GramReduceArgs rg, unsigned long long* __restrict__ stamps) {
	constexpr int TH = 128;
	unsigned long long t_loop0 = 0, t_loop1 = 0, r_loop0 = 0, r_loop1 = 0, r_entry = 0, r_tail = 0;
	if (DIAG != 0) r_entry = __builtin_amdgcn_s_memrealtime();
	extern __shared__ __attribute__((aligned(16))) float lds[];
	constexpr bool FOLD = NBW == 1;
	const int pblocks = xtiles * splits * (FOLD ? 2 : 1);
	if (blockIdx.x >= (unsigned)pblocks) {
		if (blockIdx.y != 0) return;
		if constexpr (NBW == 4) {
			if (rg.wide_P != nullptr) {
				const int pid = (int)blockIdx.x - pblocks;
				gram_wide_slice<4, false>(rg.wide_P, RP, rg.wide_len, rg.wide_parts, rg.wide_partial, pid % rg.wide_parts, pid / rg.wide_parts);
			}
			return;
		}
		if (rg.inv_a != nullptr) inverse_gj64_body<float, X3_WAVES>(rg.inv_a, 64, rg.inv_r, rg.inv_out, rg.inv_offdiag, rg.inv_diag);
		else if (rg.image != nullptr) { if (X3_WAVES == 4) gram_image_block(rg, blockIdx.x - pblocks, lds); }
		else gram_reduce_block_x3<64 * X3_WAVES>(rg, blockIdx.x - pblocks, lds);
		return;
	}
	int vb = blockIdx.x;
	if (XCD_REMAP) {
		const int q8 = pblocks / 8, r8 = pblocks % 8, xcd = vb % 8, idx = vb / 8;
		vb = (xcd < r8 ? xcd * (q8 + 1) : r8 * (q8 + 1) + (xcd - r8) * q8) + idx;
	}
	const int chunk = FOLD ? (vb & 1) : (int)blockIdx.y;
	if (FOLD) vb >>= 1;
	const int xt = vb % xtiles, sp = vb / xtiles;
	const int coff = 32 * NBW * chunk;
	const long fstep = (long)NBT * 192;
	const int wave = __builtin_amdgcn_readfirstlane(threadIdx.x >> 6);
	const int lane = threadIdx.x & 63;
	const int half = lane >> 5, l31 = lane & 31;
	const int nw = splits * X3_WAVES;
	const int widx = sp * X3_WAVES + wave;
	static_assert(!ODD || (D == 2 && !YLDS), "odd pieces: ring depth 2, loads straight to registers");
	constexpr int DU = D <= 2 ? 2 : D;
	const int units = (steps_total + DU - 1) / DU;
	const int pairs = (steps_total - nw + 1) / 2;
	const int s0 = ODD ? 2 * (int)(((long)pairs * widx) / nw) + widx : DU * (int)(((long)units * widx) / nw);
	const int s1 = ODD ? 2 * (int)(((long)pairs * (widx + 1)) / nw) + widx + 1 : DU * (int)(((long)units * (widx + 1)) / nw);
	const int steps = s1 - s0;

	f32x16 acc[4][NBW];
#pragma unroll
	for (int b = 0; b < 4; ++b)
#pragma unroll
		for (int nb = 0; nb < NBW; ++nb)
#pragma unroll
			for (int g = 0; g < 16; ++g) acc[b][nb][g] = 0.f;

	if (steps > 0) {
		const float* ap = IMG == 16 ? (TR ? A + ((long)xt * TH + (R32 ? l31 : 4 * l31)) * 16 + 8 * half
		                                  : A + ((long)xt * 8 + (l31 >> 2)) * tile_stride + (8 * half) * 16 + 4 * (l31 & 3))
		                            : (TR ? A + ((long)xt * TH + 4 * l31) * TH + 8 * half
		                                  : A + (long)xt * tile_stride + (8 * half) * TH + 4 * l31);
		auto a_addr = [&](int step, int i) -> const float* {
			if (IMG == 16) {
				if (TR) return ap + (long)step * tile_stride + (i >> 1) * (R32 ? 32 * 16 : 16) + 4 * (i & 1);
				return ap + ((long)step * 16 + i) * 16;
			}
			if (TR) return ap + (long)(step >> 3) * tile_stride + (step & 7) * 16 + (i >> 1) * TH + 4 * (i & 1);
			return ap + ((long)step * 16 + i) * TH;
		};
		const float* gp = A + (long)xt * TH * 16 + 4 * lane;
		auto g_addr = [&](int step, int i) -> const float* { return gp + (long)step * tile_stride + i * 256; };
		float* lw = lds + wave * (2 * 128 * 20);
		const int wofs = (lane >> 2) * 20 + 4 * (lane & 3);
		const int rofs = l31 * 20 + 8 * half;
		const bf16x8* fp = F + (long)chunk * (NBW * 192) + lane;
		const int last = s1 - 1, kend = steps_total - 1;
		f32x4 va[D][8];
		bf16x8 fb[D][NBW][3];
#pragma unroll
		for (int d = 0; d < D; ++d) {
			int st = s0 + (ODD ? (d ^ 1) : d);
			st = st < last ? st : last;
			const int sa = st < kend ? st : kend, sf = st <= kend ? st : steps_total;
#pragma unroll
			for (int j = 0; j < 8; ++j) va[d][j] = *reinterpret_cast<const f32x4*>(YLDS ? g_addr(sa, j) : a_addr(sa, j));
#pragma unroll
			for (int nb = 0; nb < NBW; ++nb)
#pragma unroll
				for (int pl = 0; pl < 3; ++pl) fb[d][nb][pl] = fp[(long)sf * fstep + (nb * 3 + pl) * 64];
		}
		__builtin_amdgcn_sched_barrier(0);
		if (DIAG != 0) { t_loop0 = __builtin_amdgcn_s_memtime(); r_loop0 = __builtin_amdgcn_s_memrealtime(); __builtin_amdgcn_sched_barrier(0); }
		bf16x8 op[2][3];
		f32x4 raw[2][2];
		if (YLDS) {
#pragma unroll
			for (int d = 0; d < 2; ++d) {
#pragma unroll
				for (int j = 0; j < 8; ++j) *reinterpret_cast<f32x4*>(lw + d * 2560 + j * 320 + wofs) = va[d % D][j];
				int st = s0 + D + d;
				st = st < last ? st : last;
				const int sa = st < kend ? st : kend;
#pragma unroll
				for (int j = 0; j < 8; ++j) va[d % D][j] = *reinterpret_cast<const f32x4*>(g_addr(sa, j));
			}
			raw[0][0] = *reinterpret_cast<const f32x4*>(lw + rofs); raw[0][1] = *reinterpret_cast<const f32x4*>(lw + rofs + 4);
			raw[1][0] = *reinterpret_cast<const f32x4*>(lw + 640 + rofs); raw[1][1] = *reinterpret_cast<const f32x4*>(lw + 640 + rofs + 4);
			float v[8];
#pragma unroll
			for (int j = 0; j < 4; ++j) { v[j] = raw[0][0][j]; v[4 + j] = raw[0][1][j]; }
			split3(v, op[0][0], op[0][1], op[0][2]);
		} else {
			float v[8];
#pragma unroll
			for (int j = 0; j < 8; ++j) v[j] = TR ? va[ODD ? D - 1 : 0][j >> 2][j & 3] : va[ODD ? D - 1 : 0][j][0];
			split3(v, op[0][0], op[0][1], op[0][2]);
		}
		auto kstep = [&](auto dtag, const int t) {
			constexpr int d = decltype(dtag)::value;
			{
#pragma unroll
				for (int b = 0; b < 4; ++b) {
					const int cur = (d * 4 + b) & 1, nxt = cur ^ 1;
					const int nd = b == 3 ? (d + 1) % D : d, nbk = (b + 1) & 3;
					if (YLDS) {
						float v[8];
#pragma unroll
						for (int j = 0; j < 4; ++j) { v[j] = raw[nxt][0][j]; v[4 + j] = raw[nxt][1][j]; }
						split3(v, op[nxt][0], op[nxt][1], op[nxt][2]);
						const int b2 = (b + 2) & 3;
						const int slot = (t + d + (b >= 2 ? 1 : 0)) & 1;
						const float* rp = lw + slot * 2560 + b2 * 640 + rofs;
						raw[cur][0] = *reinterpret_cast<const f32x4*>(rp); raw[cur][1] = *reinterpret_cast<const f32x4*>(rp + 4);
					} else {
						float v[8];
#pragma unroll
						for (int j = 0; j < 8; ++j) v[j] = TR ? va[nd][2 * nbk + (j >> 2)][j & 3] : va[nd][j][nbk];
						split3(v, op[nxt][0], op[nxt][1], op[nxt][2]);
					}
#pragma unroll
					for (int nb = 0; nb < NBW; ++nb) {
						acc[b][nb] = __builtin_amdgcn_mfma_f32_32x32x16_bf16(op[cur][2], fb[d][nb][0], acc[b][nb], 0, 0, 0);
						acc[b][nb] = __builtin_amdgcn_mfma_f32_32x32x16_bf16(op[cur][0], fb[d][nb][2], acc[b][nb], 0, 0, 0);
						acc[b][nb] = __builtin_amdgcn_mfma_f32_32x32x16_bf16(op[cur][1], fb[d][nb][1], acc[b][nb], 0, 0, 0);
						acc[b][nb] = __builtin_amdgcn_mfma_f32_32x32x16_bf16(op[cur][1], fb[d][nb][0], acc[b][nb], 0, 0, 0);
						acc[b][nb] = __builtin_amdgcn_mfma_f32_32x32x16_bf16(op[cur][0], fb[d][nb][1], acc[b][nb], 0, 0, 0);
						acc[b][nb] = __builtin_amdgcn_mfma_f32_32x32x16_bf16(op[cur][0], fb[d][nb][0], acc[b][nb], 0, 0, 0);
					}
					if (b == 3) {
						int st = s0 + t + D + d;
						st = st < last ? st : last;
						const int sa = st < kend ? st : kend, sf = st <= kend ? st : steps_total;
						if (YLDS) {
							const int rs = (d + 2) % D;
							const int slot = (t + d) & 1;
#pragma unroll
							for (int j = 0; j < 8; ++j) *reinterpret_cast<f32x4*>(lw + slot * 2560 + j * 320 + wofs) = va[rs][j];
							int s2 = s0 + t + d + 2 + D;
							s2 = s2 < last ? s2 : last;
							const int sa2 = s2 < kend ? s2 : kend;
#pragma unroll
							for (int j = 0; j < 8; ++j) va[rs][j] = *reinterpret_cast<const f32x4*>(g_addr(sa2, j));
						} else if (DIAG == 0 || DIAG == 2 || DIAG == 4) {
#pragma unroll
							for (int j = 0; j < 8; ++j) va[d][j] = *reinterpret_cast<const f32x4*>(a_addr(sa, j));
						} else {
#pragma unroll
							for (int j = 0; j < 8; ++j) asm volatile("" : "+v"(va[d][j]));
						}
						if (DIAG == 0 || DIAG == 3 || DIAG == 4) {
#pragma unroll
							for (int nb = 0; nb < NBW; ++nb)
#pragma unroll
								for (int pl = 0; pl < 3; ++pl) fb[d][nb][pl] = fp[(long)sf * fstep + (nb * 3 + pl) * 64];
						} else {
#pragma unroll
							for (int nb = 0; nb < NBW; ++nb)
#pragma unroll
								for (int pl = 0; pl < 3; ++pl) asm volatile("" : "+v"(fb[d][nb][pl]));
						}
						constexpr int NM = 6 * NBW, VPM = (44 + NM - 1) / NM, NL = 8 + 3 * NBW;
#pragma unroll
						for (int g = 0; g < NM; ++g) {
							__builtin_amdgcn_sched_group_barrier(0x008, 1, 0);
							__builtin_amdgcn_sched_group_barrier(0x002, VPM, 0);
							if (g < NL) __builtin_amdgcn_sched_group_barrier(0x020, 1, 0);
						}
						if (NL > NM) __builtin_amdgcn_sched_group_barrier(0x020, NL - NM, 0);
					} else {
						constexpr int NM = 6 * NBW, VPM = (44 + NM - 1) / NM;
#pragma unroll
						for (int g = 0; g < NM; ++g) {
							__builtin_amdgcn_sched_group_barrier(0x008, 1, 0);
							__builtin_amdgcn_sched_group_barrier(0x002, VPM, 0);
						}
					}
					__builtin_amdgcn_sched_barrier(0);
				}
			}
		};
#define X3_KSTEP(dd) kstep(std::integral_constant<int, dd>{}, t)
		int t = 0;
		if constexpr (ODD) { t = -1; X3_KSTEP(1); t = 1; }
		for (; t < steps; t += D) {
			X3_KSTEP(0);
			if constexpr (D > 1) X3_KSTEP(1);
			if constexpr (D > 2) X3_KSTEP(2);
			if constexpr (D > 3) X3_KSTEP(3);
			static_assert(D <= 4, "ring depth");
		}
#undef X3_KSTEP
		if (DIAG != 0) { __builtin_amdgcn_sched_barrier(0); t_loop1 = __builtin_amdgcn_s_memtime(); r_loop1 = __builtin_amdgcn_s_memrealtime(); __builtin_amdgcn_sched_barrier(0); }
	}

	if (DIAG != 0) { __builtin_amdgcn_sched_barrier(0); r_tail = __builtin_amdgcn_s_memrealtime(); __builtin_amdgcn_sched_barrier(0); }
	if (YLDS) __syncthreads();
	f32x4* l4 = reinterpret_cast<f32x4*>(lds);
	float* slab = slabs + (long)sp * slab_stride;
	constexpr int TPR = (X3_EPILOGUE_ONE_ROUND && NBW == 2 && !YLDS) ? 8 : 4;
	constexpr int ROUNDS = 4 * NBW / TPR;
#pragma unroll
	for (int rd = 0; rd < ROUNDS; ++rd) {
		if (rd > 0) __syncthreads();
#pragma unroll
		for (int tl = 0; tl < TPR; ++tl) {
			const int b = (TPR * rd + tl) / NBW, nb = (TPR * rd + tl) % NBW;
#pragma unroll
			for (int q = 0; q < 4; ++q) {
				f32x4 v;
				v[0] = acc[b][nb][4 * q + 0]; v[1] = acc[b][nb][4 * q + 1];
				v[2] = acc[b][nb][4 * q + 2]; v[3] = acc[b][nb][4 * q + 3];
				l4[((wave * TPR + tl) * 4 + q) * 64 + lane] = v;
			}
		}
		__syncthreads();
// ... 56 lines not shown
	if (hipError_t e = allow_dynamic_lds(reinterpret_cast<const void*>(&k_factor_product_x3<D, WAVES, DIAG, NBW, TR, IMG, YLDS, R32, ODD>), (int)lds_bytes, lds_done); e != hipSuccess) return e;
	if (t_ev_start != nullptr && t_ev_stop != nullptr) {
		const hipEvent_t e0 = t_ev_start, e1 = t_ev_stop;
		t_ev_start = t_ev_stop = nullptr;
		hipExtLaunchKernelGGL((k_factor_product_x3<D, WAVES, DIAG, NBW, TR, IMG, YLDS, R32, ODD>), grid, block, (std::uint32_t)lds_bytes, stream, e0, e1, 0u,
		                      A, tile_stride, reinterpret_cast<const bf16x8*>(F), RP / 32, slabs, slab_stride, RP, p.steps_total, p.xtiles, p.splits, with_reduce ? *rg : none, stamps);
		return hipGetLastError();
	}
	hipLaunchKernelGGL((k_factor_product_x3<D, WAVES, DIAG, NBW, TR, IMG, YLDS, R32, ODD>), grid, block, lds_bytes, stream,
	                   A, tile_stride, reinterpret_cast<const bf16x8*>(F), RP / 32, slabs, slab_stride, RP, p.steps_total, p.xtiles, p.splits, with_reduce ? *rg : none, stamps);
	return hipGetLastError();
}

static bool x3_odd_pieces(int steps_total, int pieces) {
	if (X3_DEAL_TURNS != 0 || X3_RING_X != 2 || pieces <= 0 || steps_total < 3 * pieces) return false;
	const int units = (steps_total + 1) / 2, pairs = (steps_total - pieces + 1) / 2;
	return 2 * ((pairs + pieces - 1) / pieces) + 1 < 2 * ((units + pieces - 1) / pieces);
}

hipError_t launch_factor_product_x3(const FactorProductPlan& p, const float* A, long tile_stride, const void* F, int RP,
                                    float* slabs, long slab_stride, hipStream_t stream, const GramReduceArgs* rg, unsigned long long* stamps,
                                    bool y_tiled, int image_tile, hipEvent_t ev_start, hipEvent_t ev_stop) {
	if (RP % 64 != 0 || p.th != 128 || (image_tile != 128 && image_tile != 16)) return hipErrorInvalidValue;
	const bool odd = x3_odd_pieces(p.steps_total, 4 * p.splits);
	t_ev_start = ev_start; t_ev_stop = ev_stop;
	struct Clear { ~Clear() { t_ev_start = t_ev_stop = nullptr; } } clear_on_exit;
#ifdef NMFAMD_DIAG_BUILD
	if (image_tile == 16 && RP == 64 && stamps != nullptr) {
		static const int yv = [] { const char* e = tuning_env("NMFAMD_X3_VARIANT"); return e ? std::atoi(e) : 0; }();
		if (!y_tiled) switch (yv % 10) {
			case 0: return (odd ? launch_fp_x3<X3_RING_X, 4, 1, 2, false, 16, false, false, true>(p, A, tile_stride, F, RP, slabs, slab_stride, stream, rg, stamps) : launch_fp_x3<X3_RING_X, 4, 1, 2, false, 16>(p, A, tile_stride, F, RP, slabs, slab_stride, stream, rg, stamps));
			case 1: return (odd ? launch_fp_x3<X3_RING_X, 4, 2, 2, false, 16, false, false, true>(p, A, tile_stride, F, RP, slabs, slab_stride, stream, rg, stamps) : launch_fp_x3<X3_RING_X, 4, 2, 2, false, 16>(p, A, tile_stride, F, RP, slabs, slab_stride, stream, rg, stamps));
			case 2: return (odd ? launch_fp_x3<X3_RING_X, 4, 3, 2, false, 16, false, false, true>(p, A, tile_stride, F, RP, slabs, slab_stride, stream, rg, stamps) : launch_fp_x3<X3_RING_X, 4, 3, 2, false, 16>(p, A, tile_stride, F, RP, slabs, slab_stride, stream, rg, stamps));
			default: return (odd ? launch_fp_x3<X3_RING_X, 4, 4, 2, false, 16, false, false, true>(p, A, tile_stride, F, RP, slabs, slab_stride, stream, rg, stamps) : launch_fp_x3<X3_RING_X, 4, 4, 2, false, 16>(p, A, tile_stride, F, RP, slabs, slab_stride, stream, rg, stamps));
		}
		switch (yv % 10) {
			case 0: return (odd ? launch_fp_x3<X3_RING_X, 4, 1, 2, true, 16, false, true, true>(p, A, tile_stride, F, RP, slabs, slab_stride, stream, rg, stamps) : launch_fp_x3<X3_RING_X, 4, 1, 2, true, 16, false, true>(p, A, tile_stride, F, RP, slabs, slab_stride, stream, rg, stamps));
			case 1: return (odd ? launch_fp_x3<X3_RING_X, 4, 2, 2, true, 16, false, true, true>(p, A, tile_stride, F, RP, slabs, slab_stride, stream, rg, stamps) : launch_fp_x3<X3_RING_X, 4, 2, 2, true, 16, false, true>(p, A, tile_stride, F, RP, slabs, slab_stride, stream, rg, stamps));
			case 2: return (odd ? launch_fp_x3<X3_RING_X, 4, 3, 2, true, 16, false, true, true>(p, A, tile_stride, F, RP, slabs, slab_stride, stream, rg, stamps) : launch_fp_x3<X3_RING_X, 4, 3, 2, true, 16, false, true>(p, A, tile_stride, F, RP, slabs, slab_stride, stream, rg, stamps));
			default: return (odd ? launch_fp_x3<X3_RING_X, 4, 4, 2, true, 16, false, true, true>(p, A, tile_stride, F, RP, slabs, slab_stride, stream, rg, stamps) : launch_fp_x3<X3_RING_X, 4, 4, 2, true, 16, false, true>(p, A, tile_stride, F, RP, slabs, slab_stride, stream, rg, stamps));
		}
	}
#else
	if (stamps != nullptr) return hipErrorNotSupported;
#endif
	if (image_tile == 16) {
		static const bool ylds = tuning_env("NMFAMD_X3_YLDS") != nullptr, ydirect = tuning_env("NMFAMD_X3_YDIRECT") != nullptr;
		if (RP % 128 == 0) {
			if (!y_tiled) return launch_fp_x3<2, 4, 0, 4, false, 16>(p, A, tile_stride, F, RP, slabs, slab_stride, stream, rg);
			return ydirect ? launch_fp_x3<2, 4, 0, 4, true, 16>(p, A, tile_stride, F, RP, slabs, slab_stride, stream, rg)
			               : launch_fp_x3<2, 4, 0, 4, true, 16, false, true>(p, A, tile_stride, F, RP, slabs, slab_stride, stream, rg);
		}
#ifdef NMFAMD_DIAG_BUILD
		if (RP == 64 && p.col_split == 2) {
			if (!y_tiled) return (odd ? launch_fp_x3<X3_RING_X, 4, 0, 1, false, 16, false, false, true>(p, A, tile_stride, F, RP, slabs, slab_stride, stream, rg) : launch_fp_x3<X3_RING_X, 4, 0, 1, false, 16>(p, A, tile_stride, F, RP, slabs, slab_stride, stream, rg));
			return (odd ? launch_fp_x3<X3_RING_X, 4, 0, 1, true, 16, false, true, true>(p, A, tile_stride, F, RP, slabs, slab_stride, stream, rg) : launch_fp_x3<X3_RING_X, 4, 0, 1, true, 16, false, true>(p, A, tile_stride, F, RP, slabs, slab_stride, stream, rg));
		}
#endif
		if (!y_tiled) return (odd ? launch_fp_x3<X3_RING_X, 4, 0, 2, false, 16, false, false, true>(p, A, tile_stride, F, RP, slabs, slab_stride, stream, rg) : launch_fp_x3<X3_RING_X, 4, 0, 2, false, 16>(p, A, tile_stride, F, RP, slabs, slab_stride, stream, rg));
		if (ylds) return launch_fp_x3<X3_RING_Y, 4, 0, 2, true, 16, true>(p, A, tile_stride, F, RP, slabs, slab_stride, stream, rg);
		if (ydirect) return (odd ? launch_fp_x3<X3_RING_X, 4, 0, 2, true, 16, false, false, true>(p, A, tile_stride, F, RP, slabs, slab_stride, stream, rg) : launch_fp_x3<X3_RING_X, 4, 0, 2, true, 16>(p, A, tile_stride, F, RP, slabs, slab_stride, stream, rg));
		return (odd ? launch_fp_x3<X3_RING_X, 4, 0, 2, true, 16, false, true, true>(p, A, tile_stride, F, RP, slabs, slab_stride, stream, rg) : launch_fp_x3<X3_RING_X, 4, 0, 2, true, 16, false, true>(p, A, tile_stride, F, RP, slabs, slab_stride, stream, rg));
	}
	if (y_tiled) {
		if (RP % 128 == 0) return launch_fp_x3<2, 4, 0, 4, true>(p, A, tile_stride, F, RP, slabs, slab_stride, stream, rg);
#ifdef NMFAMD_DIAG_BUILD
		if (RP == 64 && p.col_split == 2) return (odd ? launch_fp_x3<X3_RING_X, 4, 0, 1, true, 128, false, false, true>(p, A, tile_stride, F, RP, slabs, slab_stride, stream, rg) : launch_fp_x3<X3_RING_X, 4, 0, 1, true>(p, A, tile_stride, F, RP, slabs, slab_stride, stream, rg));
#endif
		return (odd ? launch_fp_x3<X3_RING_X, 4, 0, 2, true, 128, false, false, true>(p, A, tile_stride, F, RP, slabs, slab_stride, stream, rg) : launch_fp_x3<X3_RING_X, 4, 0, 2, true>(p, A, tile_stride, F, RP, slabs, slab_stride, stream, rg));
	}
	static const int variant = [] { const char* e = tuning_env("NMFAMD_X3_VARIANT"); return e ? std::atoi(e) : 0; }();
	if (RP == 64 && p.col_split == 2) return (odd ? launch_fp_x3<X3_RING_X, 4, 0, 1, false, 128, false, false, true>(p, A, tile_stride, F, RP, slabs, slab_stride, stream, rg) : launch_fp_x3<X3_RING_X, 4, 0, 1>(p, A, tile_stride, F, RP, slabs, slab_stride, stream, rg));
	if (RP % 128 == 0 && variant != 20) return launch_fp_x3<2, 4, 0, 4>(p, A, tile_stride, F, RP, slabs, slab_stride, stream, rg);
#ifdef NMFAMD_DIAG_BUILD
	switch (variant) {
	case 1: return launch_fp_x3<2, 4>(p, A, tile_stride, F, RP, slabs, slab_stride, stream, rg);
	case 2: return launch_fp_x3<4, 4>(p, A, tile_stride, F, RP, slabs, slab_stride, stream, rg);
	default: break;
	}
#endif
	return (odd ? launch_fp_x3<X3_RING_X, 4, 0, 2, false, 128, false, false, true>(p, A, tile_stride, F, RP, slabs, slab_stride, stream, rg) : launch_fp_x3<X3_RING_X, 4>(p, A, tile_stride, F, RP, slabs, slab_stride, stream, rg));
}

}
```

Before: 10980 iterations/s.

## Prefetch next factor-product's first V tiles into L2 from the MU update kernel

Appends extra 'passenger' blocks to the MU update kernel that load the first ring-fill steps of V (or Vt) each wave of the next x3 factor-product kernel will read, so those lines sit in L2 when that kernel starts. The block/piece/address mapping is factored into a shared header so the warm blocks reproduce the same XCD remap and step split. This is meant to hide the startup latency of the bandwidth-bound product kernel behind the small update kernel. The cost is extra blocks and memory traffic in the update launch, plus the risk of evicting other useful lines or mismatching the real access pattern.

```diff
diff --git a/nmfgpu_amd/csrc/amd_api.cpp b/nmfgpu_amd/csrc/amd_api.cpp
--- a/nmfgpu_amd/csrc/amd_api.cpp
+++ b/nmfgpu_amd/csrc/amd_api.cpp
@@ -621,7 +621,14 @@
 		const bool last = i == 39;
 		unsigned long long* sy = last && ytiled ? (unsigned long long*)dT.p : nullptr;
 		unsigned long long* sx = last && !ytiled ? (unsigned long long*)dT.p : nullptr;
+#ifdef NMFAMD_DIAG_BUILD
+		static const bool warm = tuning_env("NMFAMD_TUNE_L2_WARM") != nullptr && std::atoi(tuning_env("NMFAMD_TUNE_L2_WARM")) != 0;
+		if (warm && launch_x3_warm_alone(x3_warm_args(planH, (const float*)dA.p, stride, RP, true, 16), nullptr) != hipSuccess) return NMFAMD_HIP_ERROR;
+#endif
 		if (launch_factor_product_x3(planH, (const float*)dA.p, stride, dWx.p, RP, (float*)dS.p, slab_stride, nullptr, nullptr, sy, true, 16) != hipSuccess) return NMFAMD_HIP_ERROR;
+#ifdef NMFAMD_DIAG_BUILD
+		if (warm && launch_x3_warm_alone(x3_warm_args(planW, (const float*)dA.p, stride, RP, false, 16), nullptr) != hipSuccess) return NMFAMD_HIP_ERROR;
+#endif
 		if (launch_factor_product_x3(planW, (const float*)dA.p, stride, dHx.p, RP, (float*)dS.p, slab_stride, nullptr, nullptr, sx, false, 16) != hipSuccess) return NMFAMD_HIP_ERROR;
 	}
 	if (hipMemcpy(stamps_out, dT.p, sizeof(unsigned long long) * 8 * nwaves, hipMemcpyDeviceToHost) != hipSuccess) return NMFAMD_HIP_ERROR;
diff --git a/nmfgpu_amd/csrc/engine.cpp b/nmfgpu_amd/csrc/engine.cpp
--- a/nmfgpu_amd/csrc/engine.cpp
+++ b/nmfgpu_amd/csrc/engine.cpp
@@ -267,6 +267,7 @@
 	if (row_blocks_ > 1) { const long g = 128l * row_blocks_; mpad_ = ((mpad_ + g - 1) / g) * g; }
 	npad_ = pad128(std::max<long>(n_, (long)planH_.xtiles * planH_.th));
 	img_th_ = (one_image_ && tuning_env("NMFAMD_IMAGE_TILE128") == nullptr) ? 16 : planW_.th;
+	if (const char* e = tuning_env("NMFAMD_L2_WARM")) l2_warm_ = std::atoi(e) != 0;
 	strideV_ = (long)img_th_ * npad_;
 	strideVt_ = (long)planH_.th * mpad_;
 	elemsV_ = mpad_ * npad_;
@@ -839,7 +840,7 @@
 }
 
 template <typename T>
-Status Engine<T>::mu64_update(bool is_w, const T* slabs, int S, long slab_stride, const T* Q, bool compute_error, const PeerSlabs* peers) {
+Status Engine<T>::mu64_update(bool is_w, const T* slabs, int S, long slab_stride, const T* Q, bool compute_error, const PeerSlabs* peers, bool warm_next) {
 	if constexpr (std::is_same<T, float>::value) {
 		const float eps = std::numeric_limits<float>::epsilon();
 		float* P = is_w ? Wt_ : H_;
@@ -852,9 +853,15 @@
 		ns.off = (float)prm_.theta / (float)(unsigned)r_; ns.diag = (float)((1.0 - (float)prm_.theta) + ns.off); ns.r = r_;
 		const bool smooth = alg_ == ALG_NSNMF && !is_w;
 		if (alg_ == ALG_NSNMF && !gram_image_) return ST_INVALID;
+		X3WarmArgs wa;
+		if (warm_next && l2_warm_ && x3_ && gram_image_ && peers == nullptr && !sparse_ && !bf16_) {
+			if (!is_w) wa = x3_warm_args(planWx_, V_, strideV_, RP_, false, img_th_);
+			else if (one_image_) wa = x3_warm_args(planHx_, V_, strideV_, RP_, true, img_th_);
+			else wa = x3_warm_args(planHx_, Vt_, strideVt_, RP_, false, 128);
+		}
 		if (gram_image_) HIPX(launch_mu64_update32(is_w ? 1 : 0, P, slabs, S, slab_stride, Q, scale_, eps, ps, len, len_pad, is_w ? G_ : nullptr, compute_error ? 1 : 0, stream_, xo, xks, peers,
 		                                           is_w ? wsq_part_ : nullptr, (!is_w && (const void*)Q == (const void*)Gpart_) ? gram_ksplit_ : 0, (!is_w && (const void*)Q == (const void*)Gpart_) ? G_ : nullptr,
-		                                           smooth ? &ns : nullptr));
+		                                           smooth ? &ns : nullptr, &wa));
 		else HIPX(launch_mu64_update(is_w ? 1 : 0, P, slabs, S, slab_stride, Q, scale_, eps, ps, len, len_pad, is_w ? gramW_part_ : gramH_part_, is_w ? G_ : nullptr,
 		                             compute_error ? 1 : 0, stream_, xo, xks));
 	}
@@ -1756,10 +1763,10 @@
 		GramReduceArgs rgW = gram_args(true, G_, scale_, normalize_next_);
 		if (h_product_ahead_) h_product_ahead_ = false;
 		else if (Status s = product_h(Wt_, &rgW, x3_ && wx3_valid_)) return s;
-		if (Status s = mu64_update(false, slabs_, planH_.splits, slab_stride_, rgW.ksplit > 1 ? reinterpret_cast<const T*>(Gpart_) : G_, compute_error)) return s;
+		if (Status s = mu64_update(false, slabs_, planH_.splits, slab_stride_, rgW.ksplit > 1 ? reinterpret_cast<const T*>(Gpart_) : G_, compute_error, nullptr, true)) return s;
 		GramReduceArgs rgH = gram_args(false, HHt_, nullptr, 0);
 		if (Status s = product_w(H_, &rgH, nullptr, x3_)) return s;
-		if (Status s = mu64_update(true, slabs_, planW_.splits, slab_stride_, HHt_, compute_error)) return s;
+		if (Status s = mu64_update(true, slabs_, planW_.splits, slab_stride_, HHt_, compute_error, nullptr, true)) return s;
 		wx3_valid_ = x3_;
 		hx3_valid_ = false;
 		normalize_next_ = 1;
diff --git a/nmfgpu_amd/csrc/engine.h b/nmfgpu_amd/csrc/engine.h
--- a/nmfgpu_amd/csrc/engine.h
+++ b/nmfgpu_amd/csrc/engine.h
@@ -222,6 +222,7 @@
 	FactorProductPlan planHb_, planWb_;
 	bool x3_ = false;
 	bool one_image_ = false;
+	bool l2_warm_ = true;
 	int img_th_ = 128;
 	bool wx3_valid_ = false, hx3_valid_ = false;
 	void *Wx3_ = nullptr, *Hx3_ = nullptr;
@@ -258,7 +259,7 @@
 	bool gram_image_ = false;
 	GramReduceArgs gram_args(bool of_w, float* G, float* scale, int normalize) const;
 	Status standalone_gram(const GramReduceArgs& rg);
-	Status mu64_update(bool is_w, const T* slabs, int S, long slab_stride, const T* Q, bool compute_error, const PeerSlabs* peers = nullptr);
+	Status mu64_update(bool is_w, const T* slabs, int S, long slab_stride, const T* Q, bool compute_error, const PeerSlabs* peers = nullptr, bool warm_next = false);
 	bool gram_w_ready_ = false;
 	bool tri_ = false;
 	unsigned* tri_ride_counters_ = nullptr;
diff --git a/nmfgpu_amd/csrc/kernels.h b/nmfgpu_amd/csrc/kernels.h
--- a/nmfgpu_amd/csrc/kernels.h
+++ b/nmfgpu_amd/csrc/kernels.h
@@ -6,6 +6,8 @@
 
 #include <atomic>
 #include <vector>
+
+#include "x3_map.h"
 
 namespace nmfamd {
 
@@ -89,7 +91,7 @@
 hipError_t launch_mu64_update32(int is_w, float* P, const float* slabs, int S, long slab_stride, const float* Q, const float* scale,
                                 float eps, float* ps, int len_valid, int len_pad, const float* Gprev, int compute_error, hipStream_t stream,
                                 void* x3_out, int x3_ks, const PeerSlabs* peers = nullptr, float* colsq_part = nullptr, int qsplit = 0, float* q_out = nullptr,
-                                const SmoothAround* ns = nullptr);
+                                const SmoothAround* ns = nullptr, const X3WarmArgs* warm = nullptr);
 hipError_t launch_sum_peers(const PeerSlabs& src, float* out, int count, hipStream_t stream);
 hipError_t launch_gram_from_image(const void* image, int image_ks, float* G, float* scale, int normalize, hipStream_t stream, const float* colsq_part = nullptr, int colsq_parts = 0);
 hipError_t launch_gram_image_args(const GramReduceArgs& rg, hipStream_t stream);
@@ -289,6 +291,10 @@
                                     unsigned long long* stamps = nullptr, bool y_tiled = false, int image_tile = 128,
                                     hipEvent_t ev_start = nullptr, hipEvent_t ev_stop = nullptr);
 int plan_splits_x3(int xtiles, int KS, int num_cus, int reserve = 0);
+X3WarmArgs x3_warm_args(const FactorProductPlan& p, const float* A, long tile_stride, int RP, bool y_tiled, int image_tile);
+#ifdef NMFAMD_DIAG_BUILD
+hipError_t launch_x3_warm_alone(const X3WarmArgs& warm, hipStream_t stream);
+#endif
 
 struct OnePassArgs {
 	const float* V; long tile_stride;
diff --git a/nmfgpu_amd/csrc/kernels_mu64.hip b/nmfgpu_amd/csrc/kernels_mu64.hip
--- a/nmfgpu_amd/csrc/kernels_mu64.hip
+++ b/nmfgpu_amd/csrc/kernels_mu64.hip
@@ -4,6 +4,7 @@
 #include "kernels.h"
 #include "split3.h"
 #include "gram_image.h"
+#include "x3_map.h"
 
 namespace nmfamd {
 
@@ -181,8 +182,9 @@
 	float* __restrict__ P, const float* __restrict__ slabs, int S, long slab_stride,
 	const float* __restrict__ Q, const float* __restrict__ scale, float eps,
 	float* __restrict__ ps, int len_valid, const float* __restrict__ Gprev, int compute_error, bf16x8* __restrict__ x3_out, int x3_ks, PeerSlabs peers,
-	float* __restrict__ colsq_part, int qsplit, float* __restrict__ q_out, float ns_a_arg, float ns_b_arg, int ns_r) {
+	float* __restrict__ colsq_part, int qsplit, float* __restrict__ q_out, float ns_a_arg, float ns_b_arg, int ns_r, int ublocks, X3WarmArgs warm) {
 	static_assert(!(NS && IS_W), "the smoothing matrix rides the H update only");
+	if (blockIdx.x >= (unsigned)ublocks) { x3_warm_block(warm, (int)blockIdx.x); return; }
 	typedef float f32x4v __attribute__((ext_vector_type(4)));
 	__shared__ __attribute__((aligned(16))) float s_num[32][68];
 	__shared__ __attribute__((aligned(16))) float s_old[32][68];
@@ -355,7 +357,7 @@
 		if (l15 == 0) *reinterpret_cast<f32x4v*>(colsq_part + (long)blockIdx.x * 64 + 16 * wave + 4 * q) = sq;
 	}
 	if (IS_W && compute_error && wave == 0) {
-		for (int d = blockIdx.x; d < 64; d += gridDim.x) {
+		for (int d = blockIdx.x; d < 64; d += ublocks) {
 			float v = Q[(long)lane * 64 + d] * Gprev[(long)d * 64 + lane];
 			for (int w = 32; w > 0; w >>= 1) v += __shfl_xor(v, w);
 			if (lane == 0) ps[d] = v;
@@ -389,14 +391,16 @@
 template <bool IS_W, int U, int QS, bool NS = false>
 static void launch_update32_inst(dim3 grid, hipStream_t stream, float* P, const float* slabs, int S, long slab_stride, const float* Q, const float* scale, float eps, float* ps,
                                  int len_valid, const float* Gprev, int compute_error, bf16x8* xo, int x3_ks, const PeerSlabs& peers, float* colsq_part, float* q_out,
-                                 const SmoothAround* ns = nullptr) {
+                                 const X3WarmArgs& warm, const SmoothAround* ns = nullptr) {
+	const int ublocks = (int)grid.x;
+	if (warm.A != nullptr) grid.x = (unsigned)(warm.first + warm.xtiles * warm.splits);
 	hipLaunchKernelGGL((k_mu64_update32<IS_W, U, QS, NS>), grid, dim3(256), 0, stream, P, slabs, S, slab_stride, Q, scale, eps, ps, len_valid, Gprev, compute_error, xo, x3_ks, peers,
-	                   colsq_part, QS, q_out, NS ? ns->diag - ns->off : 1.f, NS ? ns->off : 0.f, NS ? ns->r : 0);
+	                   colsq_part, QS, q_out, NS ? ns->diag - ns->off : 1.f, NS ? ns->off : 0.f, NS ? ns->r : 0, ublocks, warm);
 }
 
 hipError_t launch_mu64_update32(int is_w, float* P, const float* slabs, int S, long slab_stride, const float* Q, const float* scale,
                                 float eps, float* ps, int len_valid, int len_pad, const float* Gprev, int compute_error, hipStream_t stream,
-                                void* x3_out, int x3_ks, const PeerSlabs* peers, float* colsq_part, int qsplit, float* q_out, const SmoothAround* ns) {
+                                void* x3_out, int x3_ks, const PeerSlabs* peers, float* colsq_part, int qsplit, float* q_out, const SmoothAround* ns, const X3WarmArgs* warm) {
 	if (x3_out == nullptr || len_pad % 32 != 0 || (qsplit > 1 && is_w) || (qsplit > 1 && qsplit != 2 && qsplit != 4 && qsplit != 8)) return hipErrorInvalidValue;
 	if (ns != nullptr && (is_w || ns->r < 1 || ns->r > 64)) return hipErrorInvalidValue;
 	PeerSlabs pa = {};
@@ -407,8 +411,13 @@
 	}
 	dim3 grid(len_pad / 32);
 	bf16x8* xo = reinterpret_cast<bf16x8*>(x3_out);
-#define NMFAMD_U32(ISW, UU, QQ) launch_update32_inst<ISW, UU, QQ>(grid, stream, P, slabs, S, slab_stride, Q, scale, eps, ps, len_valid, Gprev, compute_error, xo, x3_ks, pa, colsq_part, q_out)
-#define NMFAMD_U32NS(UU, QQ) launch_update32_inst<false, UU, QQ, true>(grid, stream, P, slabs, S, slab_stride, Q, scale, eps, ps, len_valid, Gprev, compute_error, xo, x3_ks, pa, colsq_part, q_out, ns)
+	X3WarmArgs wa;
+	if (NMFAMD_L2_WARM != 0 && warm != nullptr && warm->A != nullptr && peers == nullptr && warm->xtiles > 0 && warm->splits > 0 && warm->steps_total > 0) {
+		wa = *warm;
+		wa.first = (int)((grid.x + 7) / 8 * 8);
+	}
+#define NMFAMD_U32(ISW, UU, QQ) launch_update32_inst<ISW, UU, QQ>(grid, stream, P, slabs, S, slab_stride, Q, scale, eps, ps, len_valid, Gprev, compute_error, xo, x3_ks, pa, colsq_part, q_out, wa)
+#define NMFAMD_U32NS(UU, QQ) launch_update32_inst<false, UU, QQ, true>(grid, stream, P, slabs, S, slab_stride, Q, scale, eps, ps, len_valid, Gprev, compute_error, xo, x3_ks, pa, colsq_part, q_out, wa, ns)
 	if (ns != nullptr) {
 		if (S > 8) { if (qsplit == 2) NMFAMD_U32NS(13, 2); else if (qsplit == 4) NMFAMD_U32NS(13, 4); else if (qsplit == 8) NMFAMD_U32NS(13, 8); else NMFAMD_U32NS(13, 1); }
 		else { if (qsplit == 2) NMFAMD_U32NS(7, 2); else if (qsplit == 4) NMFAMD_U32NS(7, 4); else if (qsplit == 8) NMFAMD_U32NS(7, 8); else NMFAMD_U32NS(7, 1); }
@@ -436,6 +445,16 @@
 	hipLaunchKernelGGL(k_sum_peers, dim3((unsigned)((count / 4 + 255) / 256)), dim3(256), 0, stream, src, out, count);
 	return hipGetLastError();
 }
+
+#ifdef NMFAMD_DIAG_BUILD
+__global__ __launch_bounds__(256) void k_x3_warm_alone(X3WarmArgs warm) { x3_warm_block(warm, (int)blockIdx.x); }
+
+hipError_t launch_x3_warm_alone(const X3WarmArgs& warm, hipStream_t stream) {
+	if (warm.A == nullptr || warm.first != 0) return hipErrorInvalidValue;
+	hipLaunchKernelGGL(k_x3_warm_alone, dim3((unsigned)(warm.xtiles * warm.splits)), dim3(256), 0, stream, warm);
+	return hipGetLastError();
+}
+#endif
 
 __global__ __launch_bounds__(256) void k_gram_image(GramReduceArgs rg) {
 	__shared__ __attribute__((aligned(16))) float lds[GRAM_IMAGE_LDS_FLOATS];
diff --git a/nmfgpu_amd/csrc/kernels_x3.hip b/nmfgpu_amd/csrc/kernels_x3.hip
--- a/nmfgpu_amd/csrc/kernels_x3.hip
+++ b/nmfgpu_amd/csrc/kernels_x3.hip
@@ -12,17 +12,10 @@
 #include "inverse_gj64.h"
 #include "gram_image.h"
 #include "gram_wide.h"
+#include "x3_map.h"
 
 namespace nmfamd {
 
-#ifndef NMFAMD_XCD_REMAP
-#define NMFAMD_XCD_REMAP 1
-#endif
-constexpr bool XCD_REMAP = NMFAMD_XCD_REMAP != 0;
-
-#ifndef X3_RING_X
-#define X3_RING_X 2
-#endif
 #ifndef X3_EPILOGUE_ONE_ROUND
 #define X3_EPILOGUE_ONE_ROUND 1
 #endif
@@ -142,14 +135,8 @@
 		else gram_reduce_block_x3<64 * X3_WAVES>(rg, blockIdx.x - pblocks, lds);
 		return;
 	}
-	int vb = blockIdx.x;
-	if (XCD_REMAP) {
-		const int q8 = pblocks / 8, r8 = pblocks % 8, xcd = vb % 8, idx = vb / 8;
-		vb = (xcd < r8 ? xcd * (q8 + 1) : r8 * (q8 + 1) + (xcd - r8) * q8) + idx;
-	}
-	const int chunk = FOLD ? (vb & 1) : (int)blockIdx.y;
-	if (FOLD) vb >>= 1;
-	const int xt = vb % xtiles, sp = vb / xtiles;
+	const X3Block me = x3_block<FOLD>((int)blockIdx.x, (int)blockIdx.y, xtiles, splits);
+	const int chunk = me.chunk, xt = me.xt, sp = me.sp;
 	const int coff = 32 * NBW * chunk;
 	const long fstep = (long)NBT * 192;
 	const int wave = __builtin_amdgcn_readfirstlane(threadIdx.x >> 6);
@@ -158,11 +145,8 @@
 	const int nw = splits * X3_WAVES;
 	const int widx = sp * X3_WAVES + wave;
 	static_assert(!ODD || (D == 2 && !YLDS), "odd pieces: ring depth 2, loads straight to registers");
-	constexpr int DU = D <= 2 ? 2 : D;
-	const int units = (steps_total + DU - 1) / DU;
-	const int pairs = (steps_total - nw + 1) / 2;
-	const int s0 = ODD ? 2 * (int)(((long)pairs * widx) / nw) + widx : DU * (int)(((long)units * widx) / nw);
-	const int s1 = ODD ? 2 * (int)(((long)pairs * (widx + 1)) / nw) + widx + 1 : DU * (int)(((long)units * (widx + 1)) / nw);
+	const X3Piece piece = x3_piece<D, ODD>(widx, nw, steps_total);
+	const int s0 = piece.s0, s1 = piece.s1;
 	const int steps = s1 - s0;
 
 	f32x16 acc[4][NBW];
@@ -174,18 +158,7 @@
 			for (int g = 0; g < 16; ++g) acc[b][nb][g] = 0.f;
 
 	if (steps > 0) {
-		const float* ap = IMG == 16 ? (TR ? A + ((long)xt * TH + (R32 ? l31 : 4 * l31)) * 16 + 8 * half
-		                                  : A + ((long)xt * 8 + (l31 >> 2)) * tile_stride + (8 * half) * 16 + 4 * (l31 & 3))
-		                            : (TR ? A + ((long)xt * TH + 4 * l31) * TH + 8 * half
-		                                  : A + (long)xt * tile_stride + (8 * half) * TH + 4 * l31);
-		auto a_addr = [&](int step, int i) -> const float* {
-			if (IMG == 16) {
-				if (TR) return ap + (long)step * tile_stride + (i >> 1) * (R32 ? 32 * 16 : 16) + 4 * (i & 1);
-				return ap + ((long)step * 16 + i) * 16;
-			}
-			if (TR) return ap + (long)(step >> 3) * tile_stride + (step & 7) * 16 + (i >> 1) * TH + 4 * (i & 1);
-			return ap + ((long)step * 16 + i) * TH;
-		};
+		const X3Loads<TR, IMG, R32> a_addr(A, tile_stride, xt, lane);
 		const float* gp = A + (long)xt * TH * 16 + 4 * lane;
 		auto g_addr = [&](int step, int i) -> const float* { return gp + (long)step * tile_stride + i * 256; };
 		float* lw = lds + wave * (2 * 128 * 20);
@@ -197,9 +170,10 @@
 		bf16x8 fb[D][NBW][3];
 #pragma unroll
 		for (int d = 0; d < D; ++d) {
-			int st = s0 + (ODD ? (d ^ 1) : d);
+			int st = x3_fill_step<ODD>(s0, d);
+			const int sa = x3_clamp_a(st, last, kend);
 			st = st < last ? st : last;
-			const int sa = st < kend ? st : kend, sf = st <= kend ? st : steps_total;
+			const int sf = st <= kend ? st : steps_total;
 #pragma unroll
 			for (int j = 0; j < 8; ++j) va[d][j] = *reinterpret_cast<const f32x4*>(YLDS ? g_addr(sa, j) : a_addr(sa, j));
 #pragma unroll
@@ -267,8 +241,9 @@
 					}
 					if (b == 3) {
 						int st = s0 + t + D + d;
+						const int sa = x3_clamp_a(st, last, kend);
 						st = st < last ? st : last;
-						const int sa = st < kend ? st : kend, sf = st <= kend ? st : steps_total;
+						const int sf = st <= kend ? st : steps_total;
 						if (YLDS) {
 							const int rs = (d + 2) % D;
 							const int slot = (t + d) & 1;
@@ -491,4 +466,16 @@
 	return (odd ? launch_fp_x3<X3_RING_X, 4, 0, 2, false, 128, false, false, true>(p, A, tile_stride, F, RP, slabs, slab_stride, stream, rg) : launch_fp_x3<X3_RING_X, 4>(p, A, tile_stride, F, RP, slabs, slab_stride, stream, rg));
 }
 
-}
+X3WarmArgs x3_warm_args(const FactorProductPlan& p, const float* A, long tile_stride, int RP, bool y_tiled, int image_tile) {
+	X3WarmArgs w;
+	if (A == nullptr || RP != 64 || p.th != 128 || p.col_split == 2 || (image_tile != 128 && image_tile != 16) || p.xtiles < 1 || p.splits < 1 || p.steps_total < 1) return w;
+	if (const char* e = tuning_env("NMFAMD_X3_VARIANT")) { if (std::atoi(e) == 1 || std::atoi(e) == 2) return w; }
+	if (image_tile == 16 && y_tiled && (tuning_env("NMFAMD_X3_YLDS") != nullptr || tuning_env("NMFAMD_X3_YDIRECT") != nullptr)) return w;
+	w.A = A; w.tile_stride = tile_stride;
+	w.xtiles = p.xtiles; w.splits = p.splits; w.steps_total = p.steps_total;
+	w.tr = y_tiled ? 1 : 0; w.img16 = image_tile == 16 ? 1 : 0; w.r32 = (y_tiled && image_tile == 16) ? 1 : 0;
+	w.odd = x3_odd_pieces(p.steps_total, 4 * p.splits) ? 1 : 0;
+	return w;
+}
+
+}
diff --git a/nmfgpu_amd/csrc/x3_map.h b/nmfgpu_amd/csrc/x3_map.h
--- /dev/null
+++ b/nmfgpu_amd/csrc/x3_map.h
@@ -0,0 +1,130 @@
+#pragma once
+
+#include <hip/hip_runtime.h>
+
+namespace nmfamd {
+
+#ifndef NMFAMD_XCD_REMAP
+#define NMFAMD_XCD_REMAP 1
+#endif
+constexpr bool XCD_REMAP = NMFAMD_XCD_REMAP != 0;
+#ifndef X3_RING_X
+#define X3_RING_X 2
+#endif
+
+__host__ __device__ inline int x3_virtual_block(int block, int pblocks) {
+	if (!XCD_REMAP) return block;
+	const int q8 = pblocks / 8, r8 = pblocks % 8, xcd = block % 8, idx = block / 8;
+	return (xcd < r8 ? xcd * (q8 + 1) : r8 * (q8 + 1) + (xcd - r8) * q8) + idx;
+}
+
+struct X3Block { int xt, sp, chunk; };
+template <bool FOLD>
+__host__ __device__ inline X3Block x3_block(int block, int block_y, int xtiles, int splits) {
+	int vb = x3_virtual_block(block, xtiles * splits * (FOLD ? 2 : 1));
+	X3Block b;
+	b.chunk = FOLD ? (vb & 1) : block_y;
+	if (FOLD) vb >>= 1;
+	b.xt = vb % xtiles;
+	b.sp = vb / xtiles;
+	return b;
+}
+
+struct X3Piece { int s0, s1; };
+template <int D, bool ODD>
+__host__ __device__ inline X3Piece x3_piece(int widx, int nw, int steps_total) {
+	constexpr int DU = D <= 2 ? 2 : D;
+	const int units = (steps_total + DU - 1) / DU;
+	const int pairs = (steps_total - nw + 1) / 2;
+	X3Piece p;
+	p.s0 = ODD ? 2 * (int)(((long)pairs * widx) / nw) + widx : DU * (int)(((long)units * widx) / nw);
+	p.s1 = ODD ? 2 * (int)(((long)pairs * (widx + 1)) / nw) + widx + 1 : DU * (int)(((long)units * (widx + 1)) / nw);
+	return p;
+}
+
+template <bool ODD>
+__host__ __device__ inline int x3_fill_step(int s0, int d) { return s0 + (ODD ? (d ^ 1) : d); }
+
+__host__ __device__ inline int x3_clamp_a(int st, int last, int kend) {
+	st = st < last ? st : last;
+	return st < kend ? st : kend;
+}
+
+template <bool TR, int IMG, bool R32>
+struct X3Loads {
+	static constexpr int TH = 128;
+	const float* ap;
+	long tile_stride;
+	__host__ __device__ X3Loads(const float* A, long tile_stride_, int xt, int lane) : tile_stride(tile_stride_) {
+		const int half = lane >> 5, l31 = lane & 31;
+		ap = IMG == 16 ? (TR ? A + ((long)xt * TH + (R32 ? l31 : 4 * l31)) * 16 + 8 * half
+		                     : A + ((long)xt * 8 + (l31 >> 2)) * tile_stride + (8 * half) * 16 + 4 * (l31 & 3))
+		               : (TR ? A + ((long)xt * TH + 4 * l31) * TH + 8 * half
+		                     : A + (long)xt * tile_stride + (8 * half) * TH + 4 * l31);
+	}
+	__host__ __device__ const float* operator()(int step, int i) const {
+		if (IMG == 16) {
+			if (TR) return ap + (long)step * tile_stride + (i >> 1) * (R32 ? 32 * 16 : 16) + 4 * (i & 1);
+			return ap + ((long)step * 16 + i) * 16;
+		}
+		if (TR) return ap + (long)(step >> 3) * tile_stride + (step & 7) * 16 + (i >> 1) * TH + 4 * (i & 1);
+		return ap + ((long)step * 16 + i) * TH;
+	}
+};
+
+#ifndef NMFAMD_L2_WARM
+#define NMFAMD_L2_WARM 1
+#endif
+#ifndef NMFAMD_L2_WARM_HALF_STEPS
+#define NMFAMD_L2_WARM_HALF_STEPS 2
+#endif
+constexpr int X3_WARM_WAVES = 4;
+static_assert(NMFAMD_L2_WARM_HALF_STEPS >= 1 && NMFAMD_L2_WARM_HALF_STEPS <= 2 * X3_RING_X && NMFAMD_L2_WARM_HALF_STEPS <= 4,
+              "the passengers fetch steps the ring fill asks for, at most sixteen loads in flight per lane");
+
+struct X3WarmArgs {
+	const float* A = nullptr;
+	long tile_stride = 0;
+	int xtiles = 0, splits = 0, steps_total = 0;
+	int tr = 0, img16 = 0, r32 = 0, odd = 0;
+	int first = 0;
+};
+
+template <bool TR, int IMG, bool R32>
+__device__ inline void x3_warm_loads(const X3WarmArgs& w, int xt, int lane, const int (&step)[2]) {
+	typedef float v4 __attribute__((ext_vector_type(4)));
+	constexpr int HS = NMFAMD_L2_WARM_HALF_STEPS;
+	const X3Loads<TR, IMG, R32> a_addr(w.A, w.tile_stride, xt, lane);
+	v4 v[4 * HS];
+#pragma unroll
+	for (int h = 0; h < HS; ++h)
+#pragma unroll
+		for (int j = 0; j < 4; ++j) v[4 * h + j] = *reinterpret_cast<const v4*>(a_addr(step[h >> 1], 4 * (h & 1) + j));
+#pragma unroll
+	for (int i = 0; i < 4 * HS; ++i) asm volatile("" : : "v"(v[i]));
+}
+
+__device__ inline void x3_warm_block(const X3WarmArgs& w, int grid_index) {
+	const int block = grid_index - w.first;
+	if (w.A == nullptr || block < 0 || block >= w.xtiles * w.splits) return;
+	const int wave = __builtin_amdgcn_readfirstlane(threadIdx.x >> 6), lane = threadIdx.x & 63;
+	if (wave >= X3_WARM_WAVES) return;
+	const X3Block me = x3_block<false>(block, 0, w.xtiles, w.splits);
+	const int widx = me.sp * X3_WARM_WAVES + wave, nw = w.splits * X3_WARM_WAVES;
+	const X3Piece piece = w.odd ? x3_piece<X3_RING_X, true>(widx, nw, w.steps_total) : x3_piece<X3_RING_X, false>(widx, nw, w.steps_total);
+	if (piece.s1 <= piece.s0) return;
+	const int last = piece.s1 - 1, kend = w.steps_total - 1;
+	int step[2];
+#pragma unroll
+	for (int k = 0; k < 2; ++k) step[k] = x3_clamp_a(w.odd ? x3_fill_step<true>(piece.s0, k ^ 1) : x3_fill_step<false>(piece.s0, k), last, kend);
+	if (w.img16) {
+		if (!w.tr) x3_warm_loads<false, 16, false>(w, me.xt, lane, step);
+		else if (w.r32) x3_warm_loads<true, 16, true>(w, me.xt, lane, step);
+		else x3_warm_loads<true, 16, false>(w, me.xt, lane, step);
+	} else {
+		if (!w.tr) x3_warm_loads<false, 128, false>(w, me.xt, lane, step);
+		else x3_warm_loads<true, 128, false>(w, me.xt, lane, step);
+	}
+}
+
+}
```

After: 10820 iterations/s. 1.4% lower.
